# nicolasavru/objective-slam

Hardware: AMD Instinct MI355X
Metric: scene_ppf_votes_per_sec (higher is better)
Workload: dtype f32; 1 GPU; 5k-point model vs 100k-point scene (BASELINE.json metric config), one resident model table, Model::ppf_lookup per step; model_points=5000, scene_points=100000, ref_point_df=8, ref_points_per_gpu=12500, vote_mode=exact, parallelism=scene-ref-shard x1, exchange=single GPU

## Files before the change

include/oslam.h:

```cpp
#ifndef OSLAM_H
#define OSLAM_H

#include <stddef.h>
#include <stdint.h>

#ifdef __cplusplus
extern "C" {
#endif

#define OSLAM_OK 0
#define OSLAM_E_INVALID 1
#define OSLAM_E_DEVICE 2
#define OSLAM_E_NOMEM 3
#define OSLAM_E_NO_VOTES 4
#define OSLAM_E_LIMIT 5
#define OSLAM_E_PEER 6

#define OSLAM_VOTE_EXACT 0
#define OSLAM_VOTE_FAST 1

typedef struct oslam_params {
    unsigned ref_point_df;
    float vote_count_threshold;
    int cpu_clustering;
    int use_l1_norm;
    int use_averaged_clusters;
    int dev;
    int vote_mode;
    int shard_rank;
    int shard_world;
    unsigned max_cells;
    unsigned pose_gpu_min;
    int no_bucket_spread;
    unsigned scratch_gib;
    int pose_two_sorts;
    int vote_order;
    int reserved[1];
} oslam_params;

typedef struct oslam_stats {
    uint64_t num_scene_ppfs;
    uint64_t num_hits;
    uint64_t num_votes;
    uint64_t num_unique_votes;
    uint64_t num_model_keys;
    uint64_t num_top;
    uint32_t max_count;
    uint32_t num_emitted;
    float ms_vote;
    float ms_total;
    uint32_t vote_launches;
    float ms_vote_kernel;
    float ms_key_kernel;
    uint32_t wide_workgroups;
    uint64_t num_pairs_probed;
    uint64_t scratch_bytes;
    uint64_t num_entries_streamed;
    uint64_t num_items;
} oslam_stats;

typedef struct oslam_cell {
    uint64_t code;
    uint32_t count;
    uint32_t pad;
} oslam_cell;

typedef struct oslam_model oslam_model;
typedef struct oslam_scene oslam_scene;

int oslam_params_default(oslam_params *p);

int oslam_d_dist_from_cloud(const float *xyz, size_t n, size_t stride_bytes, float tau_d,
                            float *d_dist_out);

int oslam_model_create(const float *xyz, const float *nrm, size_t n, size_t stride_bytes,
                       float d_dist, const oslam_params *params, oslam_model **out);
void oslam_model_destroy(oslam_model *m);

int oslam_model_save(const oslam_model *m, const char *path);
int oslam_model_load(const char *path, const oslam_params *params, oslam_model **out);
int oslam_model_info(const oslam_model *m, size_t *n_points, float *d_dist, uint64_t *table_bytes);

int oslam_model_set_point_weights(oslam_model *m, const float *weights, size_t n);

int oslam_scene_create(const float *xyz, const float *nrm, size_t n, size_t stride_bytes,
                       float d_dist, unsigned ref_point_downsample_factor,
                       const oslam_params *params, oslam_scene **out);
void oslam_scene_destroy(oslam_scene *s);

int oslam_align(oslam_model *m, oslam_scene *s, float T_rowmajor[16], oslam_stats *stats);

int oslam_align_prepare(oslam_model *m, oslam_scene *s);

typedef struct oslam_db oslam_db;
int oslam_db_create(oslam_model *const *models, size_t n, oslam_db **out);
void oslam_db_destroy(oslam_db *db);
void oslam_db_destroy_with_models(oslam_db *db);
int oslam_db_align(oslam_db *db, oslam_scene *s, float *T_out, oslam_stats *stats);
int oslam_db_size(const oslam_db *db, size_t *n_models, size_t *n_groups);

int oslam_ppf_registration(const float *const *scene_xyz, const float *const *scene_nrm,
                           const size_t *scene_n, size_t n_scenes, const float *const *model_xyz,
                           const float *const *model_nrm, const size_t *model_n, size_t n_models,
                           size_t stride_bytes, const float *model_d_dists,
                           unsigned ref_point_downsample_factor, float vote_count_threshold,
                           int cpu_clustering, int use_l1_norm, int use_averaged_clusters, int devUse,
                           const float *model_weights, float *T_out);

int oslam_ht_dist(const float A[16], const float B[16], float out[2]);

int oslam_voxel_grid(const float *xyz, const float *nrm, size_t n, size_t stride_bytes, float leaf,
                     int dev, float *xyz_out, float *nrm_out, size_t cap, size_t *n_out);

typedef struct oslam_camera {
    float fx, fy, cx, cy;
    float depth_scale;
    float z_min, z_max;
    float max_jump;
} oslam_camera;
int oslam_depth_to_cloud(const void *depth, int depth_is_u16, int width, int height, const oslam_camera *cam,
// ... 563 lines not shown
int oslam_world_bricks(oslam_world *w, int32_t *keys_out, size_t cap, size_t *n_out);
int oslam_scene_from_world(oslam_world *w, oslam_volume *vol, const oslam_world_surface_params *sp, float leaf, float d_dist,
                           unsigned ref_point_downsample_factor, const oslam_params *params, oslam_scene **out,
                           size_t *n_points_out);

typedef struct oslam_world_mesh_result {
    uint32_t vertices;
    uint32_t triangles;
    uint32_t cubes;
    uint32_t bricks;
    uint32_t window_bricks;
    uint32_t launches;
    int32_t anchor[3];
    float ms_total;
} oslam_world_mesh_result;

int oslam_world_mesh(oslam_world *w, oslam_volume *vol, const oslam_world_surface_params *sp, float *xyz_out, float *nrm_out,
                     int32_t *key_out, size_t v_cap, uint32_t *tri_out, size_t t_cap, size_t *nv_out, size_t *nt_out,
                     oslam_world_mesh_result *res);

#define OSLAM_NORMALS_SWEEPS 4
typedef struct oslam_normals_params {
    float radius;
    unsigned min_neighbours;
    float viewpoint[3];
    int orient;
    float line_ratio;
    int reserved[4];
} oslam_normals_params;

typedef struct oslam_normals_result {
    uint32_t n_valid;
    uint32_t n_cells;
    float edge;
    uint32_t launches;
    float ms_total;
    float ms_grid, ms_kernel;
} oslam_normals_result;

int oslam_normals_params_default(oslam_normals_params *p);
int oslam_cloud_normals(const float *xyz, size_t n, size_t stride_bytes, const oslam_normals_params *np, int dev,
                        float *nrm_out, float *curvature_out, uint8_t *valid_out, oslam_normals_result *res);
int oslam_cloud_normal_moments(const float *xyz, size_t n, size_t stride_bytes, const oslam_normals_params *np, int dev,
                               int64_t *moments_out);
int oslam_mesh_normals(const float *xyz, size_t nv, size_t stride_bytes, const uint32_t *tri, size_t nt, float *nrm_out,
                       uint8_t *valid_out);
int oslam_ply_read_mesh(const char *path, float **xyz_out, float **nrm_out, uint32_t **tri_out, size_t *nv_out,
                        size_t *nt_out);

typedef struct oslam_colour_params {
    unsigned max_weight;
    float band;
    int reserved[6];
} oslam_colour_params;

int oslam_view_set_colour(oslam_view *v, const uint8_t *rgb, size_t row_stride_bytes, const uint8_t *valid);
int oslam_view_colour(oslam_view *v, uint32_t *rgba_out);
int oslam_view_has_colour(const oslam_view *v);
int oslam_colour_params_default(oslam_colour_params *p);
int oslam_volume_colour_enable(oslam_volume *vol, const oslam_colour_params *cp);
int oslam_volume_colour_words(oslam_volume *vol, uint32_t *words_out);
int oslam_volume_set_colour_words(oslam_volume *vol, const uint32_t *words);
int oslam_volume_integrate_colour(oslam_volume *vol, const oslam_view *v, const oslam_view *c, const float T_vol_cam[16],
                                  oslam_integrate_result *res, uint32_t *coloured_out);
int oslam_volume_colours(oslam_volume *vol, const float *xyz, size_t n, size_t stride_bytes, uint8_t *rgb_out,
                         uint8_t *valid_out, size_t *n_valid_out);
int oslam_volume_paint_view(oslam_volume *vol, const float T_vol_cam[16], oslam_view *v, uint32_t *painted_out);
int oslam_ply_write_colour(const char *path, const float *xyz, const float *nrm, const uint8_t *rgb, size_t n, int binary);
int oslam_ply_write_mesh_colour(const char *path, const float *xyz, const float *nrm, const uint8_t *rgb, size_t nv,
                                const uint32_t *tri, size_t nt, int binary);
int oslam_world_colours(oslam_world *w, oslam_volume *vol, const oslam_world_surface_params *sp, const float *xyz, size_t n,
                        size_t stride_bytes, uint8_t *rgb_out, uint8_t *valid_out, size_t *n_valid_out);

int oslam_scene_keys(oslam_scene *s, size_t ref_index, uint32_t *keys_out);
int oslam_model_keys(oslam_model *m, size_t ref_index, uint32_t *keys_out);
int oslam_model_bucket(oslam_model *m, uint32_t key, uint32_t *pairs_out, size_t cap,
                       size_t *count_out);
int oslam_model_bucket_words(oslam_model *m, uint32_t key, int slice, uint32_t *words_out, size_t cap,
                             size_t *count_out);
int oslam_model_key_numbers(oslam_model *m, uint32_t *keys_out, uint32_t *numbers_out, uint64_t *weights_out, size_t cap,
                            size_t *n_out);
int oslam_vote_ref_order(const uint32_t *keep, size_t n, uint32_t *order_out);
int oslam_vote_accumulator(oslam_model *m, oslam_scene *s, size_t ref_index, uint32_t *acc_out);
int oslam_vote_hits(oslam_model *m, oslam_scene *s, size_t ref_index, uint32_t *numbers_out, uint32_t *theta_out,
                    uint32_t *idx_out, size_t cap, size_t *n_out, uint32_t *keep_out);
int oslam_last_cells(oslam_model *m, oslam_cell *cells_out, float *poses_out, size_t cap,
                     size_t *n_out);

int oslam_set_stream(void *hip_stream);
int oslam_release_scratch(int dev);
const char *oslam_last_error(void);
int oslam_set_host_threads(int n);
int oslam_selftest_math(size_t n, uint64_t seed, uint64_t *mismatches);

#ifdef __cplusplus
}
#endif
#endif
```

objective-slam_amd/csrc/oslam_host.c:

```c
#include <pthread.h>
#include <stdio.h>

#include "oslam_internal.h"

static __thread char g_err[512];
static __thread void *g_stream;

const char *oslam_last_error(void) { return g_err; }

int oslam_set_stream(void *hip_stream)
{
    g_stream = hip_stream;
    return OSLAM_OK;
}

void *oslam_stream(void) { return g_stream; }

int oslam_fail(int code, const char *what)
{
    if (what != g_err) snprintf(g_err, sizeof g_err, "%s", what);
    return code;
}

int oslam_fail_call(const char *call, int err, const char *file, int line)
{
    snprintf(g_err, sizeof g_err, "%s: %s (%s:%d)", call, hipGetErrorString((hipError_t)err), file, line);
    return OSLAM_E_DEVICE;
}

int oslam_params_default(oslam_params *p)
{
    if (!p) return fail(OSLAM_E_INVALID, "params is NULL");
    memset(p, 0, sizeof *p);
    p->ref_point_df = 1;
    p->vote_count_threshold = 0.4f;
    p->cpu_clustering = 0;
    p->use_l1_norm = 0;
    p->use_averaged_clusters = 0;
    p->dev = 0;
    p->vote_mode = OSLAM_VOTE_EXACT;
    p->shard_rank = 0;
    p->shard_world = 1;
    p->max_cells = 1u << 22;
    p->pose_gpu_min = 0;
    p->no_bucket_spread = 0;
    p->scratch_gib = 0;
    p->vote_order = 0;
    return OSLAM_OK;
}

int oslam_d_dist_from_cloud(const float *xyz, size_t n, size_t stride_bytes, float tau_d,
                            float *d_dist_out)
{
    float lo[3], hi[3], ext;
    size_t i;
    int a;
    if (!xyz || !d_dist_out || n == 0 || stride_bytes < 12) return fail(OSLAM_E_INVALID, "bad cloud");
    for (a = 0; a < 3; a++) lo[a] = hi[a] = xyz[a];
    for (i = 1; i < n; i++) {
        const float *p = (const float *)((const char *)xyz + i * stride_bytes);
        for (a = 0; a < 3; a++) {
            if (p[a] < lo[a]) lo[a] = p[a];
            if (p[a] > hi[a]) hi[a] = p[a];
        }
    }
    ext = hi[0] - lo[0];
    if (hi[1] - lo[1] > ext) ext = hi[1] - lo[1];
    if (hi[2] - lo[2] > ext) ext = hi[2] - lo[2];
    *d_dist_out = tau_d * ext;
    return OSLAM_OK;
}

int oslam_pick_device(int dev_req, int *dev_out)
{
    int n = 0;
    hipError_t e = hipGetDeviceCount(&n);
    if (e != hipSuccess || n <= 0) return fail(OSLAM_E_DEVICE, "no HIP device available (the PPF path has no CPU fallback)");
    if (dev_req < 0) dev_req = 0;
    *dev_out = dev_req < n - 1 ? dev_req : n - 1;
    e = hipSetDevice(*dev_out);
    if (e != hipSuccess) return fail(OSLAM_E_DEVICE, hipGetErrorString(e));
    return OSLAM_OK;
}

#define DEVCACHE_SLOTS 64
#define DEVCACHE_MAX_BLOCK ((size_t)1 << 30)
typedef struct {
    void *p;
    size_t bytes;
    int dev, used;
} devblock;
static devblock g_devcache[DEVCACHE_SLOTS];
static pthread_mutex_t g_devcache_mu = PTHREAD_MUTEX_INITIALIZER;

int oslam_dev_alloc(void **out, size_t bytes)
{
    int dev = 0, i, best = -1, spare = -1;
    hipError_t e;
    size_t want;
    *out = NULL;
    if (bytes == 0) bytes = 16;
    if (hipGetDevice(&dev) != hipSuccess) return (int)hipErrorInvalidDevice;
    pthread_mutex_lock(&g_devcache_mu);
    for (i = 0; i < DEVCACHE_SLOTS; i++) {
        devblock *b = &g_devcache[i];
        if (!b->p) { if (spare < 0) spare = i; continue; }
        if (b->used || b->dev != dev || b->bytes < bytes || b->bytes > 2 * bytes + 65536) continue;
        if (best < 0 || b->bytes < g_devcache[best].bytes) best = i;
    }
    if (best >= 0) {
        g_devcache[best].used = 1;
        *out = g_devcache[best].p;
        pthread_mutex_unlock(&g_devcache_mu);
        return 0;
    }
    want = bytes <= DEVCACHE_MAX_BLOCK ? bytes + bytes / 8 + 256 : bytes;
    e = hipMalloc(out, want);
    if (e != hipSuccess) {
        (void)hipGetLastError();
        for (i = 0; i < DEVCACHE_SLOTS; i++)
            if (g_devcache[i].p && !g_devcache[i].used && g_devcache[i].dev == dev) {
                (void)hipFree(g_devcache[i].p);
                memset(&g_devcache[i], 0, sizeof g_devcache[i]);
                if (spare < 0) spare = i;
            }
        want = bytes;
        e = hipMalloc(out, want);
    }
    if (e == hipSuccess && spare >= 0 && want <= DEVCACHE_MAX_BLOCK) {
        g_devcache[spare].p = *out;
// ... 35 lines not shown
```

objective-slam_amd/csrc/oslam_internal.h:

```cpp
#ifndef OSLAM_INTERNAL_H
#define OSLAM_INTERNAL_H

#include <hip/hip_runtime_api.h>
#include <limits.h>
#include <stddef.h>
#include <stdint.h>
#include <stdlib.h>
#include <string.h>
#include <time.h>

#include "oslam.h"
#include "oslam_kernels.h"
#include "oslam_rigid.h"

typedef struct cloud_buf {
    int n;
    float *h_xyz, *h_nrm;
    float *d_soa;
    oslamk_cloud k;
} cloud_buf;

struct oslam_model {
    int dev;
    cloud_buf c;
    float d_dist, inv_d_dist;
    oslam_params params;
    oslamk_table table;
    oslamk_entries ent;
    uint32_t n_entries;
    uint64_t num_model_keys;
    float *weights;
    oslamk_counters *d_counters;
    oslamk_cell *d_out;
    uint32_t out_cap;
    oslam_cell *h_out;
    size_t n_local;
    uint32_t local_max;
    oslamk_cell *d_union;
    size_t union_cap;
    float *d_Tm16, *d_weights;
    oslam_cell *last_cells;
    float *last_poses;
    size_t n_last;
    int last_on_device;
    oslamk_cell *d_pose_cells;
    float *d_pose_T;
    size_t pose_cap;
    oslamk_slot *h_slots;
    int shared_union;
    int unusable;
    double cm[3];
    float inst_c[3], inst_extent;
    double bound_r;
    int bound_set;
};

struct oslam_scene {
    int dev;
    cloud_buf c;
    float d_dist;
    unsigned df;
    int rank, world;
    int n_ref;
    uint32_t *h_ref_idx, *d_ref_idx;
    float *d_tsg;
    float *d_Ts16;
    uint32_t *d_block;
    oslamk_order order;
    struct oslam_scene_grid *grids;
};

struct oslam_view {
    int dev;
    oslamk_view k;
    float *d_z;
    float max_jump;
    float *d_maps;
    uint32_t *d_colour;
};

struct oslam_volume {
    int dev;
    oslamk_volume k;
    oslam_volume_params p;
    int off[3];
    uint32_t *spare;
    oslamk_colour colour;
    uint32_t *colour_spare;
};

struct oslam_pyramid {
    int dev;
    unsigned n_levels;
    oslam_view *level[3];
};

struct oslam_render {
    int dev;
    oslam_view *view;
    size_t n_hyp;
    int32_t *d_labels;
    float *d_tol;
};

typedef struct db_group {
    int n;
    size_t *members;
    uint32_t *ukeys, *reach, *kmap, *uids;
} db_group;

struct oslam_db {
    int dev;
    size_t n;
// ... 166 lines not shown
```

objective-slam_amd/csrc/oslam_kernels.h:

```cpp
#ifndef OSLAM_KERNELS_H
#define OSLAM_KERNELS_H

#include <stddef.h>
#include <stdint.h>

#ifdef __cplusplus
extern "C" {
#endif

#define OSLAMK_SLICE 2046
#define OSLAMK_ROWS 1024
#define OSLAMK_NBIN 32

typedef struct oslamk_slot {
    uint32_t key;
    uint32_t start;
    uint32_t len;
    uint32_t cur;
} oslamk_slot;

typedef struct oslamk_uv {
    float uy, uz;
} oslamk_uv;

typedef struct oslamk_entries {
    uint32_t *e4;
    oslamk_uv *uv;
    uint16_t *mi;
    uint32_t *pw;
    oslamk_uv *puv;
    uint16_t *pdir;
    uint32_t n_real;
} oslamk_entries;
#define OSLAMK_PSEG 4096
#ifndef OSLAMK_PDIR_SHIFT
#define OSLAMK_PDIR_SHIFT 0
#endif
#define OSLAMK_PDIR_CELLS_RAW(m) ((m) <= 1u ? 1u : 1u << (31 - __builtin_clz((m) - 1u)))
#define OSLAMK_PDIR_CELLS(n) (OSLAMK_PDIR_CELLS_RAW((n) << OSLAMK_PDIR_SHIFT) > 4096u ? 4096u : OSLAMK_PDIR_CELLS_RAW((n) << OSLAMK_PDIR_SHIFT))

typedef struct oslamk_cloud {
    const float *px, *py, *pz, *nx, *ny, *nz;
    int n;
} oslamk_cloud;

typedef struct oslamk_order {
    const float *sx, *sy, *sz;
    const uint32_t *perm;
    const float *box;
} oslamk_order;
#define OSLAMK_ORDER_GROUP 64

typedef struct oslamk_uinfo {
    uint32_t start;
    uint32_t len;
} oslamk_uinfo;

typedef struct oslamk_table {
    oslamk_slot *slots;
    uint32_t cap;
    uint32_t shift;
    int n_slices;
    uint32_t *ukeys;
    uint32_t ucap;
    uint32_t ushift;
    uint32_t *reach;
    uint32_t reach_words;
    uint32_t *kmap;
    uint32_t kmap_bins;
    uint32_t *uids;
    uint32_t n_ids, id_bits, uinfo_stride;
    oslamk_uinfo *uinfo;
} oslamk_table;
#define OSLAMK_UWEIGHTS(t) ((unsigned long long *)((t).uids + (t).ucap))
#define OSLAMK_KMAP_NONE 0xffffffffu
#define OSLAMK_KMAP_MAX_BINS 2048

#define OSLAMK_REACH_BINS 16384

typedef struct oslamk_counters {
    unsigned long long hits;
    unsigned long long votes;
    unsigned long long nonzero_cells;
    uint32_t gmax;
    uint32_t out_count;
    uint32_t redo_count;
    uint32_t redo_total;
    unsigned long long entries;
    unsigned long long items;
    unsigned long long prof[4];
    uint32_t list_overflow;
    uint32_t pad_;
} oslamk_counters;

typedef struct oslamk_cell {
    unsigned long long code;
    uint32_t count;
    uint32_t pad;
} oslamk_cell;

int oslamk_row_keys(oslamk_cloud c, int ref, float d_dist, float inv_d_dist, uint32_t *keys_out,
                    void *stream);

int oslamk_model_count(oslamk_cloud c, float d_dist, float inv_d_dist, oslamk_table t,
                       uint32_t *n_unique, uint32_t *overflow, void *stream);
int oslamk_table_scan(oslamk_table t, uint32_t *total_out, void *stream);
int oslamk_union_build(oslamk_table t, uint32_t *n_keys, uint32_t *overflow, void *stream);
int oslamk_reach_build(oslamk_table t, float d_dist, void *stream);
int oslamk_union_weights(oslamk_table t, unsigned long long *weights, void *stream);
int oslamk_kmap_build(oslamk_table t, float d_dist, void *stream);
int oslamk_model_fill(oslamk_cloud c, float d_dist, float inv_d_dist, oslamk_table t,
                      const float *tmg, oslamk_entries ent, void *stream);

int oslamk_bucket_spread(oslamk_table t, oslamk_entries ent, void *stream);
int oslamk_bucket_psort(oslamk_table t, oslamk_entries ent, void *stream);

typedef struct oslamk_pay {
    uint32_t theta_t22;
    uint32_t idx;
} oslamk_pay;

typedef struct oslamk_run {
    uint32_t slot_r;
    uint32_t first;
} oslamk_run;
#define OSLAMK_RUN_SHIFT 26

typedef struct oslamk_vote_args {
    oslamk_cloud scene;
    const uint32_t *ref_idx;
    const float *tsg;
    int n_ref;
    float d_dist, inv_d_dist;
    oslamk_table table;
    oslamk_entries ent;
    float thresh;
    uint32_t fixed_gmax;
    oslamk_counters *counters;
    oslamk_cell *out;
    uint32_t out_cap;
    uint32_t *acc_dump;
    int dump_ref;
    int first_ref;
    int n_launch;
    int mode;
    uint32_t *keep_count;
    const uint32_t *hit_off;
    uint32_t *hit_key;
    oslamk_pay *hit_pay;
    oslamk_pay *hit_sorted;
    oslamk_run *runs;
    uint32_t *hit_count;
    uint32_t *run_count;
    uint32_t *redo;
    const uint32_t *ref_order;
    oslamk_order order;
} oslamk_vote_args;

int oslamk_uinfo_build(oslamk_table t, void *stream);

int oslamk_scene_count(const oslamk_vote_args *a, void *stream);
int oslamk_scene_hits(const oslamk_vote_args *a, void *stream);
int oslamk_sort_hits(const oslamk_vote_args *a, void *stream);
int oslamk_vote(const oslamk_vote_args *a, void *stream);
int oslamk_vote_wide(const oslamk_vote_args *a, void *stream);
int oslamk_vote_group(const oslamk_vote_args *d_all, const oslamk_vote_args *h_all, int nm, void *stream);

int oslamk_voxel_grid(oslamk_cloud c, float leaf, float *out6, uint32_t *n_out, void *stream);

int oslamk_depth_to_cloud(const void *d_img, int is_u16, int w, int h, float fx, float fy, float cx, float cy,
                          float scale, float z_min, float z_max, float max_jump, float *d_out6, uint32_t *n_out,
                          void *stream);

int oslam_dev_alloc(void **p, size_t bytes);
void oslam_dev_free(void *p);
void oslam_dev_cache_release(int dev);

int oslamk_aos6_to_soa(const float *d_in6, size_t n, float *d_soa, void *stream);

int oslamk_cluster_scores(int n, const int *cell, const uint32_t *shash, const uint32_t *sidx,
                          const float *sq, const float *st, const float *sw, float d_dist, int use_l1,
                          float *score, int whole_host, const unsigned long long *whole_dev, uint32_t *table, void *stream);
size_t oslamk_cluster_table_words(int n);

#define OSLAMK_MAX_INSTANCES 64
typedef struct oslamk_inst_args {
    uint32_t max_instances;
    float ratio, sep2, cos_thr;
    int32_t rot_on;
    float c[3];
} oslamk_inst_args;
typedef struct oslamk_inst_out {
    uint32_t n;
    uint32_t idx[OSLAMK_MAX_INSTANCES];
    float score[OSLAMK_MAX_INSTANCES];
    float T[OSLAMK_MAX_INSTANCES][16];
} oslamk_inst_out;

// ... 361 lines not shown
```

objective-slam_amd/csrc/oslam_kernels.hip:

```cpp
#include <hip/hip_runtime.h>

#include "oslam_kernels.h"
#include "ppf_core.h"

#include "oslam_vote_body.inc"

__device__ __forceinline__ uint32_t slot_of(uint32_t key, uint32_t shift)
{
    return (key * 2654435761u) >> shift;
}

__device__ __forceinline__ uint32_t cloud_pair_key(const oslamk_cloud &c, int i, float prx,
                                                   float pry, float prz, float nrx, float nry,
                                                   float nrz, float nrn, float d_dist,
                                                   float inv_d_dist, float *pix, float *piy,
                                                   float *piz)
{
    float px = c.px[i], py = c.py[i], pz = c.pz[i];
    float nx = c.nx[i], ny = c.ny[i], nz = c.nz[i];
    *pix = px;
    *piy = py;
    *piz = pz;
    return pc_pair_key(prx, pry, prz, nrx, nry, nrz, nrn, px, py, pz, nx, ny, nz,
                       pc_norm3(nx, ny, nz), d_dist, inv_d_dist);
// ... 246 lines not shown
                key[i] = ((unsigned long long)spread_key(w) << 32) | i;
            } else {
                key[i] = ~0ull;
            }
        }
        __syncthreads();
        for (uint32_t k = 2; k <= P; k <<= 1) {
            for (uint32_t j = k >> 1; j > 0; j >>= 1) {
                for (uint32_t x = tid; x < P / 2; x += SPREAD_THREADS) {
                    const uint32_t lo = ((x & ~(j - 1)) << 1) | (x & (j - 1)), hi = lo | j;
                    const unsigned long long a = key[lo], b = key[hi];
                    const bool up = (lo & k) == 0;
                    if ((a > b) == up) { key[lo] = b; key[hi] = a; }
                }
                __syncthreads();
            }
        }
        const uint32_t n_full = n >> 8, n_last = n & 255u;
        for (uint32_t p = tid; p < n; p += SPREAD_THREADS) {
            const uint32_t c = p >> 8, q = p & 255u, h = (q >> 2) & 31u;
            const uint32_t nc = c < n_full ? 256u : n_last;
            uint32_t rank = 8u * h * n_full + spread_rank_in_chunk(4u * h, n_last);
            rank += 8u * (c < n_full ? c : n_full);
            rank += spread_rank_in_chunk(q, nc) - spread_rank_in_chunk(4u * h, nc);
            const uint32_t src = (uint32_t)key[rank];
            ent.e4[base + p] = s_e4[src];
            if (ent.uv) ent.uv[base + p] = s_uv[src];
            ent.mi[base + p] = s_mi[src];
        }
        __syncthreads();
    }
}

__global__ __launch_bounds__(SPREAD_THREADS) void k_bucket_psort(oslamk_table t, oslamk_entries ent)
{
    __shared__ unsigned long long key[OSLAMK_PSEG];
    __shared__ uint32_t s_e4[OSLAMK_PSEG];
    __shared__ oslamk_uv s_uv[OSLAMK_PSEG];
    const oslamk_slot sl = t.slots[blockIdx.x];
    if (sl.key == 0 || sl.len == 0) return;
    const int tid = threadIdx.x;
    for (uint32_t seg = 0; seg < sl.len; seg += OSLAMK_PSEG) {
        const uint32_t n = sl.len - seg < OSLAMK_PSEG ? sl.len - seg : OSLAMK_PSEG;
        const size_t base = (size_t)sl.start + seg;
        uint32_t P = 2;
        while (P < n) P <<= 1;
        for (uint32_t i = tid; i < P; i += SPREAD_THREADS) {
            if (i < n) {
                const uint32_t w = ent.e4[base + i];
                s_e4[i] = w;
                s_uv[i] = ent.uv[base + i];
                key[i] = ((unsigned long long)(w * 30u) << 32) | i;
            } else {
                key[i] = ~0ull;
            }
        }
        __syncthreads();
        for (uint32_t k = 2; k <= P; k <<= 1) {
            for (uint32_t j = k >> 1; j > 0; j >>= 1) {
                for (uint32_t x = tid; x < P / 2; x += SPREAD_THREADS) {
                    const uint32_t lo = ((x & ~(j - 1)) << 1) | (x & (j - 1)), hi = lo | j;
                    const unsigned long long a = key[lo], b = key[hi];
                    const bool up = (lo & k) == 0;
                    if ((a > b) == up) { key[lo] = b; key[hi] = a; }
                }
                __syncthreads();
            }
        }
        for (uint32_t i = tid; i < n; i += SPREAD_THREADS) {
            const uint32_t src = (uint32_t)key[i];
            ent.pw[base + i] = s_e4[src];
            ent.puv[base + i] = s_uv[src];
        }
        const uint32_t K = OSLAMK_PDIR_CELLS(n);
        for (uint32_t k = tid; k <= K; k += SPREAD_THREADS) {
            uint32_t lo = 0, hi = n;
            while (lo < hi) {
                const uint32_t mid = (lo + hi) >> 1;
                const uint32_t cell = (uint32_t)(((key[mid] >> 32) * (unsigned long long)K) >> 32);
                if (cell < k) lo = mid + 1; else hi = mid;
            }
            ent.pdir[(base << OSLAMK_PDIR_SHIFT) + k] = (uint16_t)lo;
        }
        __syncthreads();
    }
}

#define KEY_TILE 4096
#define COUNT_REFS 8
#define HIT_TILE 1024

__device__ const uint32_t d_acos_lut[2 * PC_ACOS_CELLS] = {PC_ACOS_LUT_FLAT};

__device__ __forceinline__ int pair_dist_bin_quick(float dx, float dy, float dz, float d_dist, float inv_d_dist)
{
    const float d2 = dx * dx + dy * dy + dz * dz;
    const float q = __builtin_amdgcn_sqrtf(d2) * inv_d_dist;
    const float kf = __builtin_floorf(q);
    const float fr = q - kf, tol = q * 1e-6f;
    int k = (int)kf;
    if (!(d2 > 1e-30f && q < 1048576.0f && fr > tol && 1.0f - fr > tol)) k = pc_pair_dist_bin(dx, dy, dz, d_dist, inv_d_dist);
    return k;
}

__device__ __forceinline__ bool bin_in_reach(const uint32_t *reach, uint32_t reach_words, int k)
{
    if ((uint32_t)k >= OSLAMK_REACH_BINS) return true;
    const uint32_t w = (uint32_t)k >> 5;
    return w < reach_words && ((reach[w] >> ((uint32_t)k & 31u)) & 1u);
}

struct KeyRefs {
    uint32_t rr[COUNT_REFS];
    float prx[COUNT_REFS], pry[COUNT_REFS], prz[COUNT_REFS];
};
__device__ __forceinline__ void key_refs_load(KeyRefs &r, const oslamk_vote_args &a, int g0)
{
#pragma unroll
    for (int g = 0; g < COUNT_REFS; g++) {
        const bool v = g0 + g < a.n_launch;
        r.rr[g] = v ? a.ref_idx[a.first_ref + g0 + g] : 0xffffffffu;
        r.prx[g] = v ? a.scene.px[r.rr[g]] : 0.0f;
        r.pry[g] = v ? a.scene.py[r.rr[g]] : 0.0f;
        r.prz[g] = v ? a.scene.pz[r.rr[g]] : 0.0f;
    }
}
__device__ __forceinline__ void reach_fill(uint32_t *s_reach, const uint32_t *reach, uint32_t reach_words)
{
    for (uint32_t w = threadIdx.x; w < reach_words; w += 256) s_reach[w] = reach[w];
}
__device__ __forceinline__ bool pair_keep(const KeyRefs &r, int g, bool valid, int i, bool in, float x, float y, float z,
                                          const oslamk_vote_args &a, const uint32_t *s_reach, uint32_t reach_words)
{
    const int k = pair_dist_bin_quick(x - r.prx[g], y - r.pry[g], z - r.prz[g], a.d_dist, a.inv_d_dist);
    return in && (uint32_t)i != r.rr[g] && valid && bin_in_reach(s_reach, reach_words, k);
}

__device__ __forceinline__ bool range_in_reach(const uint32_t *reach, uint32_t reach_words, int kmin, int kmax)
{
    if (kmax >= OSLAMK_REACH_BINS) return true;
    const uint32_t w0 = (uint32_t)kmin >> 5, w1 = (uint32_t)kmax >> 5;
    for (uint32_t w = w0; w <= w1 && w < reach_words; w++) {
        uint32_t m = reach[w];
        if (w == w0) m &= 0xffffffffu << ((uint32_t)kmin & 31u);
        if (w == w1) m &= 0xffffffffu >> (31u - ((uint32_t)kmax & 31u));
        if (m) return true;
    }
    return false;
}
__device__ __forceinline__ bool group_keep(const oslamk_vote_args &a, int g, int grp, const uint32_t *s_reach, uint32_t reach_words)
{
    if (g >= a.n_launch || grp * OSLAMK_ORDER_GROUP >= a.scene.n) return false;
#ifdef KEY_DIAG_KEEP_ALL
    return true;
#endif
    const uint32_t rr = a.ref_idx[a.first_ref + g];
    int kmin, kmax;
    if (!pc_box_bin_range(a.order.box + 6 * (size_t)grp, a.scene.px[rr], a.scene.py[rr], a.scene.pz[rr], a.inv_d_dist, &kmin, &kmax))
        return true;
    return range_in_reach(s_reach, reach_words, kmin, kmax);
}

__global__ __launch_bounds__(256) void k_scene_count(oslamk_vote_args a)
{
    __shared__ uint32_t s_cnt[COUNT_REFS];
    __shared__ uint32_t s_reach[OSLAMK_REACH_BINS / 32];
// ... 325 lines not shown
        for (int k = 0; k < 4; k++) {
            if ((uint32_t)k >= G) continue;
            float v = votes;
            if (whole) {
                float s = lane_sum[k];
                for (int o = WAVE / 2; o > 0; o >>= 1) s += __shfl_xor(s, o, WAVE);
                v = 1 + s;
            }
            if (lane == 0) score[orig[k]] = v;
        }
        g0 += G;
    }
}

__global__ void k_selftest(const float *x, const float *y, const float *x2, size_t n, float *out_acos,
                           float *out_atan2, uint32_t *out_quant, uint32_t *out_bin)
{
    __shared__ uint32_t s_tbl[32];
    if (threadIdx.x < 32) s_tbl[threadIdx.x] = k_alpha_thr[threadIdx.x];
    __syncthreads();
    size_t i = (size_t)blockIdx.x * blockDim.x + threadIdx.x;
    if (i >= n) return;
    out_acos[i] = pm_acosf(x[i]);
    out_atan2[i] = pm_atan2f(y[i], x2[i]);
    out_quant[i] = pc_quant_bits(pm_fabsf(y[i]) * 7.0f, 0.0371f + pm_fabsf(x[i]) * 0.01f,
                                 1.0f / (0.0371f + pm_fabsf(x[i]) * 0.01f));
    out_bin[i] = pc_alpha_bin_table(y[i], x2[i], x[i], y[i] - x2[i], s_tbl);
}

extern "C" {

int oslamk_row_keys(oslamk_cloud c, int ref, float d_dist, float inv_d_dist, uint32_t *keys_out,
                    void *stream)
{
    hipLaunchKernelGGL(k_row_keys, dim3((c.n + 255) / 256), dim3(256), 0, (hipStream_t)stream, c, ref,
                       d_dist, inv_d_dist, keys_out);
    return (int)hipGetLastError();
}

int oslamk_model_count(oslamk_cloud c, float d_dist, float inv_d_dist, oslamk_table t,
                       uint32_t *n_unique, uint32_t *overflow, void *stream)
{
    hipLaunchKernelGGL(k_model_count, dim3((c.n + 255) / 256, c.n), dim3(256), 0, (hipStream_t)stream,
                       c, d_dist, inv_d_dist, t, n_unique, overflow);
    return (int)hipGetLastError();
}

int oslamk_table_scan(oslamk_table t, uint32_t *total_out, void *stream)
{
    hipLaunchKernelGGL(k_table_scan, dim3(1), dim3(1024), 0, (hipStream_t)stream, t, total_out);
    return (int)hipGetLastError();
}

int oslamk_union_build(oslamk_table t, uint32_t *n_keys, uint32_t *overflow, void *stream)
{
    size_t total = (size_t)t.n_slices * t.cap;
    hipLaunchKernelGGL(k_union_build, dim3((unsigned)((total + 255) / 256)), dim3(256), 0,
                       (hipStream_t)stream, t, n_keys, overflow);
    return (int)hipGetLastError();
}

int oslamk_model_fill(oslamk_cloud c, float d_dist, float inv_d_dist, oslamk_table t,
                      const float *tmg, oslamk_entries ent, void *stream)
{
    hipLaunchKernelGGL(k_model_fill, dim3((c.n + 255) / 256, c.n), dim3(256), 0, (hipStream_t)stream,
                       c, d_dist, inv_d_dist, t, tmg, ent);
    return (int)hipGetLastError();
}

int oslamk_bucket_spread(oslamk_table t, oslamk_entries ent, void *stream)
{
    const size_t total = (size_t)t.n_slices * t.cap;
    hipLaunchKernelGGL(k_bucket_spread, dim3((unsigned)total), dim3(SPREAD_THREADS), 0, (hipStream_t)stream, t, ent);
    return (int)hipGetLastError();
}

int oslamk_bucket_psort(oslamk_table t, oslamk_entries ent, void *stream)
{
    const size_t total = (size_t)t.n_slices * t.cap;
    hipLaunchKernelGGL(k_bucket_psort, dim3((unsigned)total), dim3(SPREAD_THREADS), 0, (hipStream_t)stream, t, ent);
    return (int)hipGetLastError();
}

int oslamk_reach_build(oslamk_table t, float d_dist, void *stream)
{
    hipLaunchKernelGGL(k_reach_build, dim3(OSLAMK_REACH_BINS), dim3(256), 0, (hipStream_t)stream, t, d_dist);
    return (int)hipGetLastError();
}

int oslamk_union_weights(oslamk_table t, unsigned long long *weights, void *stream)
{
    const size_t total = (size_t)t.n_slices * t.cap;
    hipLaunchKernelGGL(k_union_weights, dim3((unsigned)((total + 255) / 256)), dim3(256), 0, (hipStream_t)stream, t, weights);
    return (int)hipGetLastError();
}

int oslamk_kmap_build(oslamk_table t, float d_dist, void *stream)
{
    if (t.kmap_bins == 0) return 0;
    hipLaunchKernelGGL(k_kmap_build, dim3(t.kmap_bins), dim3(256), 0, (hipStream_t)stream, t, d_dist);
    return (int)hipGetLastError();
}

int oslamk_uinfo_build(oslamk_table t, void *stream)
{
    const size_t total = (size_t)t.n_slices * t.cap;
    hipLaunchKernelGGL(k_uinfo_build, dim3((unsigned)((total + 255) / 256)), dim3(256), 0, (hipStream_t)stream, t);
    return (int)hipGetLastError();
}

int oslamk_scene_count(const oslamk_vote_args *a, void *stream)
{
    if (a->n_launch <= 0) return 0;
    dim3 grid((unsigned)((a->n_launch + COUNT_REFS - 1) / COUNT_REFS), (unsigned)((a->scene.n + KEY_TILE - 1) / KEY_TILE));
    hipLaunchKernelGGL(k_scene_count, grid, dim3(256), 0, (hipStream_t)stream, *a);
    return (int)hipGetLastError();
}

int oslamk_scene_hits(const oslamk_vote_args *a, void *stream)
{
    if (a->n_launch <= 0) return 0;
    dim3 grid((unsigned)((a->n_launch + COUNT_REFS - 1) / COUNT_REFS), (unsigned)((a->scene.n + HIT_TILE - 1) / HIT_TILE));
    hipLaunchKernelGGL(k_scene_hits, grid, dim3(256), 0, (hipStream_t)stream, *a);
    return (int)hipGetLastError();
}


int oslamk_vote(const oslamk_vote_args *a, void *stream)
{
    if (a->n_launch <= 0) return 0;
    dim3 grid((unsigned)(((size_t)a->n_launch + 7) / 8 * 8 * a->table.n_slices));
    hipLaunchKernelGGL((a->mode == 0 ? k_vote<0> : k_vote<1>), grid, dim3(VOTE_THREADS), 0, (hipStream_t)stream, *a);
    return oslamk_vote_wide(a, stream);
}

int oslamk_vote_group(const oslamk_vote_args *d_all, const oslamk_vote_args *h_all, int nm, void *stream)
{
    if (nm <= 0 || h_all[0].n_launch <= 0) return 0;
    int max_slices = 1;
    for (int j = 0; j < nm; j++) {
        if (h_all[j].n_launch != h_all[0].n_launch || h_all[j].mode != h_all[0].mode) return (int)hipErrorInvalidValue;
        if (h_all[j].table.n_slices > max_slices) max_slices = h_all[j].table.n_slices;
    }
    const size_t wgs = ((size_t)h_all[0].n_launch + 7) / 8 * 8 * (size_t)max_slices;
    if (wgs * (size_t)nm > 0x7fffffffu) return (int)hipErrorInvalidValue;
    hipLaunchKernelGGL((h_all[0].mode == 0 ? k_vote_group<0> : k_vote_group<1>), dim3((unsigned)(wgs * (size_t)nm)),
                       dim3(VOTE_THREADS), 0, (hipStream_t)stream, d_all, (uint32_t)wgs);
    return (int)hipGetLastError();
}

size_t oslamk_cluster_table_words(int n)
{
    uint32_t cap = 64;
    while (cap < 2u * (uint32_t)(n > 0 ? n : 1)) cap <<= 1;
    return 3u * (size_t)cap;
}

int oslamk_cluster_scores(int n, const int *cell, const uint32_t *shash, const uint32_t *sidx,
                          const float *sq, const float *st, const float *sw, float d_dist, int use_l1,
                          float *score, int whole_host, const unsigned long long *whole_dev, uint32_t *table, void *stream)
{
    if (n <= 0) return 0;
    const size_t words = oslamk_cluster_table_words(n);
    const uint32_t mask = (uint32_t)(words / 3u) - 1u;
    hipError_t e = hipMemsetAsync(table, 0, sizeof(uint32_t) * words, (hipStream_t)stream);
    if (e != hipSuccess) return (int)e;
// ... 34 lines not shown
```

objective-slam_amd/csrc/oslam_model.c:

```c
#include <stdio.h>

#include "oslam_internal.h"
#include "oslam_pose.h"
#include "ppf_core.h"

void oslam_model_destroy(oslam_model *m)
{
    if (!m) return;
    (void)hipSetDevice(m->dev);
    oslam_cloud_free(&m->c);
    if (m->table.slots) (void)hipFree(m->table.slots);
    if (m->ent.e4) (void)hipFree(m->ent.e4);
    if (m->ent.uv) (void)hipFree(m->ent.uv);
    if (m->ent.pw) (void)hipFree(m->ent.pw);
    if (m->ent.puv) (void)hipFree(m->ent.puv);
    if (m->ent.pdir) (void)hipFree(m->ent.pdir);
    if (m->ent.mi) (void)hipFree(m->ent.mi);
    if (m->table.ukeys && !m->shared_union) (void)hipFree(m->table.ukeys);
    if (m->table.reach && !m->shared_union) (void)hipFree(m->table.reach);
    if (m->table.kmap && !m->shared_union) (void)hipFree(m->table.kmap);
    if (m->table.uids && !m->shared_union) (void)hipFree(m->table.uids);
    if (m->d_counters) (void)hipFree(m->d_counters);
    if (m->d_out) (void)hipFree(m->d_out);
    if (m->d_union) (void)hipFree(m->d_union);
    if (m->table.uinfo) (void)hipFree(m->table.uinfo);
    if (m->d_Tm16) (void)hipFree(m->d_Tm16);
    if (m->d_weights) (void)hipFree(m->d_weights);
    if (m->d_pose_cells) (void)hipFree(m->d_pose_cells);
    if (m->d_pose_T) (void)hipFree(m->d_pose_T);
    free(m->h_out);
    free(m->weights);
    free(m->last_cells);
    free(m->last_poses);
    free(m->h_slots);
    free(m);
}

typedef struct key_rank {
    uint64_t weight;
    uint32_t key, slot;
} key_rank;

static void rank_pass(const key_rank *src, key_rank *dst, size_t n, int by_weight, unsigned shift, uint32_t *count)
{
    size_t i;
    uint32_t run = 0, d;
    memset(count, 0, sizeof(uint32_t) * 65536);
    for (i = 0; i < n; i++) {
        d = by_weight ? 0xffffu - (uint32_t)((src[i].weight >> shift) & 0xffffu) : (src[i].key >> shift) & 0xffffu;
        count[d]++;
    }
    for (d = 0; d < 65536; d++) {
        const uint32_t c = count[d];
        count[d] = run;
        run += c;
    }
    for (i = 0; i < n; i++) {
        d = by_weight ? 0xffffu - (uint32_t)((src[i].weight >> shift) & 0xffffu) : (src[i].key >> shift) & 0xffffu;
        dst[count[d]++] = src[i];
    }
}

static key_rank *rank_keys(key_rank *r, key_rank *tmp, size_t n, uint32_t *count)
{
    uint64_t top = 0;
    unsigned shift;
    size_t i;
    key_rank *t;
    for (i = 0; i < n; i++) if (r[i].weight > top) top = r[i].weight;
    for (shift = 0; shift < 32; shift += 16) {
        rank_pass(r, tmp, n, 0, shift, count);
        t = r; r = tmp; tmp = t;
    }
    for (shift = 0; shift < 64 && (top >> shift); shift += 16) {
        rank_pass(r, tmp, n, 1, shift, count);
        t = r; r = tmp; tmp = t;
    }
    return r;
}

int oslam_build_kmap(oslamk_table *t, float d_dist, const oslamk_table *parts, int n_parts, int vote_order)
{
    int rc = OSLAM_OK, j;
    uint32_t h_reach[OSLAMK_REACH_BINS / 32], w, top = 0, n_ids = 0, slot;
    uint32_t *h_keys = NULL, *h_ids = NULL, *count = NULL;
    uint64_t *h_w = NULL;
    key_rank *r = NULL, *r2 = NULL, *res;
    const size_t ucap = t->ucap;
    const int ranked = vote_order == 0 || vote_order == 2;
    t->kmap = NULL;
    t->kmap_bins = 0;
    t->reach_words = 0;
    t->uids = NULL;
    t->n_ids = t->id_bits = t->uinfo_stride = 0;
    HIPCHK(hipMalloc((void **)&t->uids, (sizeof(uint32_t) + sizeof(uint64_t)) * ucap));
    HIPCHK(hipMemsetAsync(t->uids, 0, (sizeof(uint32_t) + sizeof(uint64_t)) * ucap, (hipStream_t)oslam_stream()));
    for (j = 0; j < n_parts; j++) {
        oslamk_table p = parts[j];
        p.ukeys = t->ukeys;
// ... 18 lines not shown
        for (slot = 0; slot < ucap; slot++)
            if (h_keys[slot] != 0u) {
                r[i].weight = h_w[slot];
                r[i].key = h_keys[slot];
                r[i].slot = slot;
                i++;
            }
        res = rank_keys(r, r2, n_ids, count);
        for (i = 0; i < n_ids; i++) h_ids[res[i].slot] = (uint32_t)i;
    } else {
        uint32_t next = 0;
        for (slot = 0; slot < ucap; slot++)
            if (h_keys[slot] != 0u) h_ids[slot] = next++;
    }
    HIPCHK(hipMemcpy(t->uids, h_ids, sizeof(uint32_t) * ucap, hipMemcpyHostToDevice));
    t->n_ids = n_ids;
    t->id_bits = 1;
    while (t->id_bits < 32u && ((uint64_t)1 << t->id_bits) < (uint64_t)n_ids) t->id_bits++;
    t->uinfo_stride = (n_ids + 63u) & ~63u;
    if (t->uinfo_stride == 0) t->uinfo_stride = 64;
    HIPCHK(hipMemcpy(h_reach, t->reach, sizeof h_reach, hipMemcpyDeviceToHost));
    for (w = 0; w < OSLAMK_REACH_BINS / 32; w++)
        if (h_reach[w]) {
            t->reach_words = w + 1;
            top = 32u * w + (32u - (uint32_t)__builtin_clz(h_reach[w]));
        }
    t->kmap_bins = top < OSLAMK_KMAP_MAX_BINS ? top : OSLAMK_KMAP_MAX_BINS;
    if (t->kmap_bins) {
        HIPCHK(hipMalloc((void **)&t->kmap, sizeof(uint32_t) * (size_t)t->kmap_bins * PC_ANGLE_COMBOS));
        KCHK(oslamk_kmap_build(*t, d_dist, oslam_stream()));
    }
done:
    free(h_keys);
    free(h_ids);
    free(h_w);
    free(count);
    free(r);
    free(r2);
    return rc;
}

int oslam_build_union(oslam_model *m, uint32_t distinct, uint32_t *d_n_keys, uint32_t *d_overflow)
{
    int rc = OSLAM_OK;
    uint32_t lg = 16;
    while ((1u << lg) < 4u * distinct && lg < OSLAMK_RUN_SHIFT) lg++;
    if ((1u << lg) < 2u * distinct) return fail(OSLAM_E_LIMIT, "more distinct pair keys than the union table can index");
    if (m->table.ukeys && !m->shared_union) (void)hipFree(m->table.ukeys);
    if (m->table.reach && !m->shared_union) (void)hipFree(m->table.reach);
    if (m->table.kmap && !m->shared_union) (void)hipFree(m->table.kmap);
    if (m->table.uids && !m->shared_union) (void)hipFree(m->table.uids);
    m->table.ukeys = NULL;
    m->table.reach = NULL;
    m->table.kmap = NULL;
    m->table.uids = NULL;
    m->shared_union = 0;
    m->table.ucap = 1u << lg;
    m->table.ushift = 32 - lg;
    HIPCHK(hipMalloc((void **)&m->table.ukeys, sizeof(uint32_t) * (size_t)m->table.ucap));
    HIPCHK(hipMemsetAsync(m->table.ukeys, 0, sizeof(uint32_t) * (size_t)m->table.ucap, (hipStream_t)oslam_stream()));
    HIPCHK(hipMemsetAsync(d_overflow, 0, sizeof(uint32_t), (hipStream_t)oslam_stream()));
    HIPCHK(hipMemsetAsync(d_n_keys, 0, sizeof(uint32_t), (hipStream_t)oslam_stream()));
    KCHK(oslamk_union_build(m->table, d_n_keys, d_overflow, oslam_stream()));
    HIPCHK(hipMalloc((void **)&m->table.reach, sizeof(uint32_t) * (OSLAMK_REACH_BINS / 32)));
    HIPCHK(hipMemsetAsync(m->table.reach, 0, sizeof(uint32_t) * (OSLAMK_REACH_BINS / 32), (hipStream_t)oslam_stream()));
    KCHK(oslamk_reach_build(m->table, m->d_dist, oslam_stream()));
    rc = oslam_build_kmap(&m->table, m->d_dist, &m->table, 1, m->params.vote_order);
done:
    return rc;
}

int oslam_build_uinfo(oslam_model *m)
{
    int rc = OSLAM_OK;
    const size_t bytes = sizeof(oslamk_uinfo) * (size_t)m->table.n_slices * (size_t)m->table.uinfo_stride;
    if (m->table.uinfo) { (void)hipFree(m->table.uinfo); m->table.uinfo = NULL; }
    HIPCHK(hipMalloc((void **)&m->table.uinfo, bytes));
    HIPCHK(hipMemsetAsync(m->table.uinfo, 0, bytes, (hipStream_t)oslam_stream()));
    KCHK(oslamk_uinfo_build(m->table, oslam_stream()));
done:
    return rc;
}

int oslam_model_create(const float *xyz, const float *nrm, size_t n, size_t stride_bytes,
                       float d_dist, const oslam_params *params, oslam_model **out)
{
    int rc = OSLAM_OK;
    oslam_model *m = NULL;
    uint32_t *d_small = NULL;
    uint32_t h_small[64 + 3];
    float *h_tmg = NULL, *d_tmg = NULL;
    int n_slices, s;
    uint32_t cap;
    size_t n_pairs;

    if (!out) return fail(OSLAM_E_INVALID, "out is NULL");
    *out = NULL;
    if (!xyz || !nrm || stride_bytes < 12 || !(d_dist > 0.0f)) return fail(OSLAM_E_INVALID, "bad model arguments");
    if (n < 2) return fail(OSLAM_E_INVALID, "model needs at least 2 points");
    if (n > 46340) return fail(OSLAM_E_LIMIT, "model larger than 46340 points (32-bit pair index, kernel.cu:433)");
    m = (oslam_model *)calloc(1, sizeof *m);
    if (!m) return fail(OSLAM_E_NOMEM, "host allocation failed");
    if (params) m->params = *params; else oslam_params_default(&m->params);
    if (m->params.max_cells == 0) m->params.max_cells = 1u << 22;
    rc = oslam_pick_device(m->params.dev, &m->dev);
    if (rc != OSLAM_OK) goto done;
    rc = oslam_cloud_make(&m->c, xyz, nrm, stride_bytes, NULL, n);
    if (rc != OSLAM_OK) goto done;
    oslam_cloud_shape(m->c.h_xyz, n, m->cm, m->inst_c, &m->inst_extent);
    m->d_dist = d_dist;
    m->inv_d_dist = 1.0f / d_dist;
    m->weights = (float *)malloc(sizeof(float) * n);
    if (!m->weights) { rc = fail(OSLAM_E_NOMEM, "host allocation failed"); goto done; }
    for (s = 0; s < (int)n; s++) m->weights[s] = 1.0f;

    n_slices = (int)((n + OSLAMK_SLICE - 1) / OSLAMK_SLICE);
    if (n_slices > 64) { rc = fail(OSLAM_E_LIMIT, "too many model slices"); goto done; }
    HIPCHK(hipMalloc((void **)&d_small, sizeof(uint32_t) * (64 + 3)));

    for (cap = 1u << 16;; cap <<= 1) {
        int grow = 0;
        uint32_t lg = 0;
        while ((1u << lg) < cap) lg++;
        if (m->table.slots) { (void)hipFree(m->table.slots); m->table.slots = NULL; }
        HIPCHK(hipMalloc((void **)&m->table.slots, sizeof(oslamk_slot) * (size_t)cap * n_slices));
        HIPCHK(hipMemsetAsync(m->table.slots, 0, sizeof(oslamk_slot) * (size_t)cap * n_slices, (hipStream_t)oslam_stream()));
        HIPCHK(hipMemsetAsync(d_small, 0, sizeof(uint32_t) * (64 + 3), (hipStream_t)oslam_stream()));
        m->table.cap = cap;
        m->table.shift = 32 - lg;
        m->table.n_slices = n_slices;
        KCHK(oslamk_model_count(m->c.k, m->d_dist, m->inv_d_dist, m->table, d_small, d_small + 64, oslam_stream()));
        HIPCHK(hipStreamSynchronize((hipStream_t)oslam_stream()));
        HIPCHK(hipMemcpy(h_small, d_small, sizeof h_small, hipMemcpyDeviceToHost));
        if (h_small[64]) grow = 1;
        for (s = 0; s < n_slices; s++) if (h_small[s] > cap / 2) grow = 1;
        if (!grow) break;
        if (cap >= (1u << 26)) { rc = fail(OSLAM_E_LIMIT, "model hash table would exceed 2^26 slots per slice"); goto done; }
    }
    KCHK(oslamk_table_scan(m->table, d_small + 65, oslam_stream()));
    {
        uint32_t sum = 0;
        for (s = 0; s < n_slices; s++) sum += h_small[s];
        rc = oslam_build_union(m, sum, d_small + 66, d_small + 64);
        if (rc != OSLAM_OK) goto done;
    }
    HIPCHK(hipStreamSynchronize((hipStream_t)oslam_stream()));
    HIPCHK(hipMemcpy(h_small, d_small, sizeof h_small, hipMemcpyDeviceToHost));
    if (h_small[64]) { rc = fail(OSLAM_E_LIMIT, "union key table overflow"); goto done; }
    m->n_entries = h_small[65];
    m->ent.n_real = m->n_entries;
    m->num_model_keys = (uint64_t)h_small[66] + 1;
    n_pairs = m->n_entries ? m->n_entries : 1;

    h_tmg = (float *)malloc(sizeof(float) * 8 * n);
    if (!h_tmg) { rc = fail(OSLAM_E_NOMEM, "host allocation failed"); goto done; }
    oslam_T_g_rows(m->c.h_xyz, m->c.h_nrm, NULL, n, h_tmg);
    HIPCHK(hipMalloc((void **)&d_tmg, sizeof(float) * 8 * n));
    HIPCHK(hipMemcpy(d_tmg, h_tmg, sizeof(float) * 8 * n, hipMemcpyHostToDevice));
    HIPCHK(hipMalloc((void **)&m->ent.e4, sizeof(uint32_t) * (n_pairs + 256)));
    HIPCHK(hipMalloc((void **)&m->ent.mi, sizeof(uint16_t) * n_pairs));
    if (m->params.vote_mode != OSLAM_VOTE_FAST)
        HIPCHK(hipMalloc((void **)&m->ent.uv, sizeof(oslamk_uv) * n_pairs));
    HIPCHK(hipMemsetD32Async((hipDeviceptr_t)m->ent.e4, (int)PC_ROW_SINK, n_pairs + 256, (hipStream_t)oslam_stream()));
    KCHK(oslamk_model_fill(m->c.k, m->d_dist, m->inv_d_dist, m->table, d_tmg, m->ent, oslam_stream()));
    if (!m->params.no_bucket_spread) KCHK(oslamk_bucket_spread(m->table, m->ent, oslam_stream()));
    if (m->ent.uv) {
        HIPCHK(hipMalloc((void **)&m->ent.pw, sizeof(uint32_t) * n_pairs));
        HIPCHK(hipMalloc((void **)&m->ent.puv, sizeof(oslamk_uv) * n_pairs));
        HIPCHK(hipMalloc((void **)&m->ent.pdir, sizeof(uint16_t) * ((n_pairs + 256) << OSLAMK_PDIR_SHIFT)));
        KCHK(oslamk_bucket_psort(m->table, m->ent, oslam_stream()));
        HIPCHK(hipStreamSynchronize((hipStream_t)oslam_stream()));
        (void)hipFree(m->ent.uv);
        m->ent.uv = NULL;
    }
    rc = oslam_build_uinfo(m);
    if (rc != OSLAM_OK) goto done;
    HIPCHK(hipStreamSynchronize((hipStream_t)oslam_stream()));

    m->out_cap = m->params.max_cells;
    HIPCHK(hipMalloc((void **)&m->d_counters, sizeof(oslamk_counters)));
    HIPCHK(hipMalloc((void **)&m->d_out, sizeof(oslamk_cell) * (size_t)m->out_cap));
    m->h_out = (oslam_cell *)malloc(sizeof(oslam_cell) * (size_t)m->out_cap);
    if (!m->h_out) { rc = fail(OSLAM_E_NOMEM, "host allocation failed"); goto done; }
done:
    free(h_tmg);
    if (d_tmg) (void)hipFree(d_tmg);
    if (d_small) (void)hipFree(d_small);
    if (rc != OSLAM_OK) { oslam_model_destroy(m); return rc; }
    *out = m;
    return OSLAM_OK;
}

#define OSLAM_DB_MAGIC 0x4c444d4f534c4f00ull
#define OSLAM_DB_VERSION 7u
typedef struct db_header {
    uint64_t magic;
    uint32_t version, vote_mode;
    uint32_t n_points, n_slices, cap, shift, ucap, ushift, n_entries, has_uv;
    uint64_t num_model_keys;
    float d_dist, inv_d_dist;
    uint64_t checksum;
} db_header;

static uint64_t fnv64(uint64_t h, const void *p, size_t n)
{
    const unsigned char *b = (const unsigned char *)p;
    size_t i;
    for (i = 0; i < n; i++) { h ^= b[i]; h *= 0x100000001b3ull; }
    return h;
}

static int db_write_dev(FILE *f, const void *dev, size_t bytes, uint64_t *sum)
{
    int rc = OSLAM_OK;
    const size_t chunk = (size_t)64 << 20;
    char *h = (char *)malloc(bytes < chunk ? (bytes ? bytes : 1) : chunk);
    size_t off;
    if (!h) return fail(OSLAM_E_NOMEM, "host allocation failed");
    for (off = 0; off < bytes; off += chunk) {
        const size_t n = bytes - off < chunk ? bytes - off : chunk;
        HIPCHK(hipMemcpy(h, (const char *)dev + off, n, hipMemcpyDeviceToHost));
        *sum = fnv64(*sum, h, n);
        if (fwrite(h, 1, n, f) != n) { rc = fail(OSLAM_E_INVALID, "short write"); goto done; }
    }
done:
    free(h);
    return rc;
}

static int db_read_dev(FILE *f, void *dev, size_t bytes, uint64_t *sum)
{
    int rc = OSLAM_OK;
    const size_t chunk = (size_t)64 << 20;
    char *h = (char *)malloc(bytes < chunk ? (bytes ? bytes : 1) : chunk);
    size_t off;
    if (!h) return fail(OSLAM_E_NOMEM, "host allocation failed");
    for (off = 0; off < bytes; off += chunk) {
        const size_t n = bytes - off < chunk ? bytes - off : chunk;
        if (fread(h, 1, n, f) != n) { rc = fail(OSLAM_E_INVALID, "model file is truncated"); goto done; }
        *sum = fnv64(*sum, h, n);
        HIPCHK(hipMemcpy((char *)dev + off, h, n, hipMemcpyHostToDevice));
    }
done:
    free(h);
    return rc;
}

static uint32_t log2_exact(uint32_t v)
{
    uint32_t lg = 0;
    while ((1u << lg) < v) lg++;
    return lg;
}
// ... 72 lines not shown
        hd.ucap > (1u << OSLAMK_RUN_SHIFT) || hd.shift != 32u - log2_exact(hd.cap) || hd.ushift != 32u - log2_exact(hd.ucap) ||
        !(hd.d_dist > 0.0f) || hd.inv_d_dist != 1.0f / hd.d_dist || hd.has_uv > 1u ||
        hd.vote_mode > (uint32_t)OSLAM_VOTE_FAST || (hd.vote_mode != (uint32_t)OSLAM_VOTE_FAST && !hd.has_uv) ||
        (uint64_t)hd.n_entries > (uint64_t)n * (n - 1) + 3ull * (uint64_t)hd.cap * hd.n_slices ||
        hd.num_model_keys > (uint64_t)hd.ucap + 1) {
        rc = fail(OSLAM_E_INVALID, "model file header is inconsistent");
        goto done;
    }
    hz = hd;
    hz.checksum = 0;
    sum = fnv64(sum, &hz, sizeof hz);
    m = (oslam_model *)calloc(1, sizeof *m);
    if (!m) { rc = fail(OSLAM_E_NOMEM, "host allocation failed"); goto done; }
    if (params) m->params = *params; else oslam_params_default(&m->params);
    if (m->params.max_cells == 0) m->params.max_cells = 1u << 22;
    if (params && (uint32_t)params->vote_mode != hd.vote_mode && !(hd.has_uv && params->vote_mode == OSLAM_VOTE_FAST)) {
        rc = fail(OSLAM_E_INVALID, "model file was built in fast vote mode: it has no exact entries");
        goto done;
    }
    if (!params) m->params.vote_mode = (int)hd.vote_mode;
    rc = oslam_pick_device(m->params.dev, &m->dev);
    if (rc != OSLAM_OK) goto done;
    xyz = (float *)malloc(12 * n);
    nrm = (float *)malloc(12 * n);
    m->weights = (float *)malloc(4 * n);
    n_slots = (size_t)hd.cap * hd.n_slices;
    h_slots = (oslamk_slot *)malloc(sizeof(oslamk_slot) * n_slots);
    if (!xyz || !nrm || !m->weights || !h_slots) { rc = fail(OSLAM_E_NOMEM, "host allocation failed"); goto done; }
    if (fread(xyz, 12, n, f) != n || fread(nrm, 12, n, f) != n || fread(m->weights, 4, n, f) != n ||
        fread(h_slots, sizeof(oslamk_slot), n_slots, f) != n_slots) {
        rc = fail(OSLAM_E_INVALID, "model file is truncated");
        goto done;
    }
    sum = fnv64(sum, xyz, 12 * n);
    sum = fnv64(sum, nrm, 12 * n);
    sum = fnv64(sum, m->weights, 4 * n);
    sum = fnv64(sum, h_slots, sizeof(oslamk_slot) * n_slots);
    {
        uint64_t run = 0;
        for (i = 0; i < n_slots; i++) {
            if (h_slots[i].start != run || run + h_slots[i].len > hd.n_entries) {
                rc = fail(OSLAM_E_INVALID, "model file: a bucket lies outside the entry arrays or out of order");
                goto done;
            }
            run += ((uint64_t)h_slots[i].len + 3u) & ~(uint64_t)3u;
        }
    }
    rc = oslam_cloud_make(&m->c, xyz, nrm, 12, NULL, n);
    if (rc != OSLAM_OK) goto done;
    oslam_cloud_shape(m->c.h_xyz, n, m->cm, m->inst_c, &m->inst_extent);
    m->d_dist = hd.d_dist;
    m->inv_d_dist = hd.inv_d_dist;
    m->table.cap = hd.cap;
    m->table.shift = hd.shift;
    m->table.n_slices = (int)hd.n_slices;
    m->table.ucap = hd.ucap;
    m->table.ushift = hd.ushift;
    m->n_entries = hd.n_entries;
    m->ent.n_real = hd.n_entries;
    m->num_model_keys = hd.num_model_keys;
    n_pairs = hd.n_entries ? hd.n_entries : 1;
    HIPCHK(hipMalloc((void **)&m->table.slots, sizeof(oslamk_slot) * n_slots));
    HIPCHK(hipMalloc((void **)&m->table.ukeys, sizeof(uint32_t) * (size_t)hd.ucap));
    HIPCHK(hipMalloc((void **)&m->table.reach, sizeof(uint32_t) * (OSLAMK_REACH_BINS / 32)));
    HIPCHK(hipMalloc((void **)&m->ent.e4, sizeof(uint32_t) * (n_pairs + 256)));
    HIPCHK(hipMalloc((void **)&m->ent.mi, sizeof(uint16_t) * n_pairs));
    if (hd.has_uv) {
        HIPCHK(hipMalloc((void **)&m->ent.pw, sizeof(uint32_t) * n_pairs));
        HIPCHK(hipMalloc((void **)&m->ent.puv, sizeof(oslamk_uv) * n_pairs));
        HIPCHK(hipMalloc((void **)&m->ent.pdir, sizeof(uint16_t) * ((n_pairs + 256) << OSLAMK_PDIR_SHIFT)));
    }
    HIPCHK(hipMemcpy(m->table.slots, h_slots, sizeof(oslamk_slot) * n_slots, hipMemcpyHostToDevice));
    HIPCHK(hipMemsetD32Async((hipDeviceptr_t)m->ent.e4, (int)PC_ROW_SINK, n_pairs + 256, (hipStream_t)oslam_stream()));
    HIPCHK(hipStreamSynchronize((hipStream_t)oslam_stream()));
    rc = db_read_dev(f, m->table.ukeys, sizeof(uint32_t) * (size_t)hd.ucap, &sum);
    if (rc == OSLAM_OK) rc = db_read_dev(f, m->table.reach, sizeof(uint32_t) * (OSLAMK_REACH_BINS / 32), &sum);
    if (rc == OSLAM_OK) rc = db_read_dev(f, m->ent.e4, sizeof(uint32_t) * (size_t)hd.n_entries, &sum);
    if (rc == OSLAM_OK) rc = db_read_dev(f, m->ent.mi, sizeof(uint16_t) * (size_t)hd.n_entries, &sum);
    if (rc == OSLAM_OK && hd.has_uv) rc = db_read_dev(f, m->ent.pw, sizeof(uint32_t) * (size_t)hd.n_entries, &sum);
    if (rc == OSLAM_OK && hd.has_uv) rc = db_read_dev(f, m->ent.puv, sizeof(oslamk_uv) * (size_t)hd.n_entries, &sum);
    if (rc == OSLAM_OK && hd.has_uv) rc = db_read_dev(f, m->ent.pdir, sizeof(uint16_t) * ((size_t)hd.n_entries << OSLAMK_PDIR_SHIFT), &sum);
    if (rc != OSLAM_OK) goto done;
    if (sum != hd.checksum) { rc = fail(OSLAM_E_INVALID, "model file checksum mismatch"); goto done; }
    m->h_slots = h_slots;
    h_slots = NULL;
    rc = oslam_build_kmap(&m->table, m->d_dist, &m->table, 1, m->params.vote_order);
    if (rc != OSLAM_OK) goto done;
    rc = oslam_build_uinfo(m);
    if (rc != OSLAM_OK) goto done;
    HIPCHK(hipStreamSynchronize((hipStream_t)oslam_stream()));
    m->out_cap = m->params.max_cells;
    HIPCHK(hipMalloc((void **)&m->d_counters, sizeof(oslamk_counters)));
    HIPCHK(hipMalloc((void **)&m->d_out, sizeof(oslamk_cell) * (size_t)m->out_cap));
    m->h_out = (oslam_cell *)malloc(sizeof(oslam_cell) * (size_t)m->out_cap);
    if (!m->h_out) { rc = fail(OSLAM_E_NOMEM, "host allocation failed"); goto done; }
done:
    if (f) fclose(f);
    free(xyz);
    free(nrm);
    free(h_slots);
    if (rc != OSLAM_OK) { oslam_model_destroy(m); return rc; }
    *out = m;
    return OSLAM_OK;
}

int oslam_model_info(const oslam_model *m, size_t *n_points, float *d_dist, uint64_t *table_bytes)
{
    if (!m) return fail(OSLAM_E_INVALID, "NULL handle");
    if (n_points) *n_points = (size_t)m->c.n;
    if (d_dist) *d_dist = m->d_dist;
    if (table_bytes)
        *table_bytes = sizeof(oslamk_slot) * (uint64_t)m->table.cap * (uint64_t)m->table.n_slices +
                       sizeof(uint32_t) * (uint64_t)m->table.ucap + sizeof(uint32_t) * (OSLAMK_REACH_BINS / 32) +
                       sizeof(oslamk_uinfo) * (uint64_t)m->table.uinfo_stride * (uint64_t)m->table.n_slices +
                       (uint64_t)m->n_entries * (4 + 2 + (m->ent.pw ? 12 + (2 << OSLAMK_PDIR_SHIFT) : 0)) + 24ull * (uint64_t)m->c.n;
    return OSLAM_OK;
}

int oslam_model_set_point_weights(oslam_model *m, const float *weights, size_t n)
{
    if (!m || !weights || n != (size_t)m->c.n) return fail(OSLAM_E_INVALID, "bad weights");
    memcpy(m->weights, weights, sizeof(float) * n);
    if (m->d_weights) {
        if (hipSetDevice(m->dev) != hipSuccess ||
            hipMemcpy(m->d_weights, m->weights, sizeof(float) * n, hipMemcpyHostToDevice) != hipSuccess)
            return fail(OSLAM_E_DEVICE, "cannot update the weights on the device");
    }
    return OSLAM_OK;
}
```

objective-slam_amd/csrc/oslam_taps.c:

```c

#include "oslam_internal.h"
#include "oslam_pose.h"
#include "ppf_core.h"

static int cloud_row_keys(cloud_buf *c, size_t ref, float d_dist, uint32_t *keys_out)
{
    int rc = OSLAM_OK;
    uint32_t *d = NULL;
    if (!keys_out || ref >= (size_t)c->n) return fail(OSLAM_E_INVALID, "bad reference index");
    HIPCHK(hipMalloc((void **)&d, sizeof(uint32_t) * c->n));
    KCHK(oslamk_row_keys(c->k, (int)ref, d_dist, 1.0f / d_dist, d, oslam_stream()));
    HIPCHK(hipStreamSynchronize((hipStream_t)oslam_stream()));
    HIPCHK(hipMemcpy(keys_out, d, sizeof(uint32_t) * c->n, hipMemcpyDeviceToHost));
done:
    if (d) (void)hipFree(d);
    return rc;
}

int oslam_scene_keys(oslam_scene *s, size_t ref_index, uint32_t *keys_out)
{
    if (!s) return fail(OSLAM_E_INVALID, "NULL handle");
    if (!(s->d_dist > 0.0f)) return fail(OSLAM_E_INVALID, "this scene was made for models of any d_dist (d_dist 0): it has no keys of its own");
    if (hipSetDevice(s->dev) != hipSuccess) return fail(OSLAM_E_DEVICE, "hipSetDevice failed");
    return cloud_row_keys(&s->c, ref_index, s->d_dist, keys_out);
// ... 112 lines not shown
    h_w = (uint64_t *)malloc(sizeof(uint64_t) * ucap);
    rows = (key_row *)malloc(sizeof *rows * ucap);
    if (!h_keys || !h_ids || !h_w || !rows) { rc = fail(OSLAM_E_NOMEM, "host allocation failed"); goto done; }
    HIPCHK(hipMemcpy(h_keys, m->table.ukeys, sizeof(uint32_t) * ucap, hipMemcpyDeviceToHost));
    HIPCHK(hipMemcpy(h_ids, m->table.uids, sizeof(uint32_t) * ucap, hipMemcpyDeviceToHost));
    HIPCHK(hipMemcpy(h_w, OSLAMK_UWEIGHTS(m->table), sizeof(uint64_t) * ucap, hipMemcpyDeviceToHost));
    for (slot = 0; slot < ucap; slot++)
        if (h_keys[slot] != 0u) {
            rows[n].key = h_keys[slot];
            rows[n].number = h_ids[slot];
            rows[n].weight = h_w[slot];
            n++;
        }
    qsort(rows, n, sizeof *rows, key_row_order);
    for (i = 0; i < n && i < cap; i++) {
        if (keys_out) keys_out[i] = rows[i].key;
        if (numbers_out) numbers_out[i] = rows[i].number;
        if (weights_out) weights_out[i] = rows[i].weight;
    }
    *n_out = n;
done:
    free(h_keys);
    free(h_ids);
    free(h_w);
    free(rows);
    return rc;
}

int oslam_vote_ref_order(const uint32_t *keep, size_t n, uint32_t *order_out)
{
    if ((!keep || !order_out) && n) return fail(OSLAM_E_INVALID, "NULL argument");
    oslam_ref_order(keep, n, order_out);
    return OSLAM_OK;
}

static int tap_one_ref(oslam_model *m, oslam_scene *s, size_t ref_index, uint32_t *acc_out, uint32_t *numbers_out,
                       uint32_t *theta_out, uint32_t *idx_out, size_t cap, size_t *n_out, uint32_t *keep_out)
{
    int rc = OSLAM_OK;
    uint32_t *d_dump = NULL, *d_ref = NULL, *h_dump = NULL;
    float *d_tsg = NULL;
    float rows[8];
    uint32_t ref = (uint32_t)ref_index;
    oslamk_counters cnt;
    scratch_pool *pool = NULL;
    size_t cells;
    rc = oslam_check_pair(m, s);
    if (rc != OSLAM_OK) return rc;
    if (ref_index >= (size_t)s->c.n) return fail(OSLAM_E_INVALID, "bad reference index");
    cells = (size_t)m->table.n_slices * OSLAMK_SLICE * OSLAMK_NBIN;
    oslam_T_g_rows(s->c.h_xyz, s->c.h_nrm, &ref, 1, rows);
    rc = oslam_pool_enter(m->dev, &pool);
    if (rc != OSLAM_OK) return rc;
    HIPCHK(hipMalloc((void **)&d_dump, sizeof(uint32_t) * cells));
    HIPCHK(hipMalloc((void **)&d_ref, sizeof(uint32_t)));
    HIPCHK(hipMalloc((void **)&d_tsg, sizeof rows));
    HIPCHK(hipMemcpy(d_ref, &ref, sizeof ref, hipMemcpyHostToDevice));
    HIPCHK(hipMemcpy(d_tsg, rows, sizeof rows, hipMemcpyHostToDevice));
    rc = oslam_run_votes_group(pool, &m, 1, s, d_ref, d_tsg, 1, 0xffffffffu, d_dump, &cnt, NULL);
    if (rc != OSLAM_OK) goto done;
    if (n_out) {
        rc = oslam_pool_read_hits(pool, numbers_out, theta_out, idx_out, cap, n_out, keep_out);
        if (rc != OSLAM_OK) goto done;
    }
    if (acc_out) {
        h_dump = (uint32_t *)malloc(sizeof(uint32_t) * cells);
        if (!h_dump) { rc = fail(OSLAM_E_NOMEM, "host allocation failed"); goto done; }
        HIPCHK(hipMemcpy(h_dump, d_dump, sizeof(uint32_t) * cells, hipMemcpyDeviceToHost));
        memcpy(acc_out, h_dump, sizeof(uint32_t) * OSLAMK_NBIN * (size_t)m->c.n);
    }
done:
    oslam_pool_unlock(pool);
    free(h_dump);
    if (d_dump) (void)hipFree(d_dump);
    if (d_ref) (void)hipFree(d_ref);
    if (d_tsg) (void)hipFree(d_tsg);
    return rc;
}

int oslam_vote_accumulator(oslam_model *m, oslam_scene *s, size_t ref_index, uint32_t *acc_out)
{
    if (!acc_out) return fail(OSLAM_E_INVALID, "bad reference index");
    return tap_one_ref(m, s, ref_index, acc_out, NULL, NULL, NULL, 0, NULL, NULL);
}

int oslam_vote_hits(oslam_model *m, oslam_scene *s, size_t ref_index, uint32_t *numbers_out, uint32_t *theta_out,
                    uint32_t *idx_out, size_t cap, size_t *n_out, uint32_t *keep_out)
{
    if (!n_out) return fail(OSLAM_E_INVALID, "NULL argument");
    *n_out = 0;
    return tap_one_ref(m, s, ref_index, NULL, numbers_out, theta_out, idx_out, cap, n_out, keep_out);
}

static int materialise_last(oslam_model *m)
{
    int rc = OSLAM_OK;
    const size_t n = m->n_last;
    if (!m->last_on_device) return OSLAM_OK;
    if (hipSetDevice(m->dev) != hipSuccess) return fail(OSLAM_E_DEVICE, "hipSetDevice failed");
    m->last_cells = (oslam_cell *)malloc(sizeof(oslam_cell) * (n ? n : 1));
    m->last_poses = (float *)malloc(sizeof(float) * 16 * (n ? n : 1));
    if (!m->last_cells || !m->last_poses) { oslam_drop_last(m); return fail(OSLAM_E_NOMEM, "host allocation failed"); }
    HIPCHK(hipMemcpy(m->last_cells, m->d_pose_cells, sizeof(oslam_cell) * n, hipMemcpyDeviceToHost));
    HIPCHK(hipMemcpy(m->last_poses, m->d_pose_T, sizeof(float) * 16 * n, hipMemcpyDeviceToHost));
    m->last_on_device = 0;
done:
    return rc;
}

int oslam_last_result(oslam_model *m, oslam_scene *s, float *trans_out, float *rots_out, float *vote_counts_out,
                      size_t cap, size_t *n_out, uint32_t *max_idx_out)
{
    int rc;
    size_t n;
    float T[16], *tr = NULL, *ro = NULL, *sc = NULL;
    uint32_t best = 0;
    if (!n_out) return fail(OSLAM_E_INVALID, "NULL argument");
    *n_out = 0;
    rc = oslam_check_pair(m, s);
    if (rc != OSLAM_OK) return rc;
    if (materialise_last(m) != OSLAM_OK) return OSLAM_E_DEVICE;
    n = m->n_last;
    if (max_idx_out) *max_idx_out = 0;
    if (n == 0) return OSLAM_OK;
    tr = (float *)calloc(3 * n, sizeof(float));
    ro = (float *)calloc(4 * n, sizeof(float));
    sc = (float *)calloc(n, sizeof(float));
    if (!tr || !ro || !sc) { rc = fail(OSLAM_E_NOMEM, "host allocation failed"); goto done; }
    rc = oslam_pose_stage_ex(m->last_cells, n, m->c.h_xyz, m->c.h_nrm, (size_t)m->c.n, s->c.h_xyz, s->c.h_nrm, (size_t)s->c.n,
                             m->d_dist, m->params.cpu_clustering, m->params.use_l1_norm, m->params.use_averaged_clusters,
                             m->weights, T, NULL, tr, ro, sc, &best);
    if (rc != OSLAM_OK) { rc = fail(rc, "pose stage failed"); goto done; }
    if (n > cap) n = cap;
    if (trans_out) memcpy(trans_out, tr, sizeof(float) * 3 * n);
    if (rots_out) memcpy(rots_out, ro, sizeof(float) * 4 * n);
    if (vote_counts_out) memcpy(vote_counts_out, sc, sizeof(float) * n);
    if (max_idx_out) *max_idx_out = best;
    *n_out = n;
done:
    free(tr);
    free(ro);
    free(sc);
    return rc;
}

int oslam_last_cells(oslam_model *m, oslam_cell *cells_out, float *poses_out, size_t cap, size_t *n_out)
{
    size_t n;
    if (!m || !n_out) return fail(OSLAM_E_INVALID, "NULL argument");
    if ((cells_out || poses_out) && materialise_last(m) != OSLAM_OK) return OSLAM_E_DEVICE;
    n = m->n_last < cap ? m->n_last : cap;
    if (cells_out) memcpy(cells_out, m->last_cells, sizeof(oslam_cell) * n);
    if (poses_out) memcpy(poses_out, m->last_poses, sizeof(float) * 16 * n);
    *n_out = m->n_last;
    return OSLAM_OK;
}

static uint64_t sm64(uint64_t *s)
{
    uint64_t z = (*s += 0x9e3779b97f4a7c15ull);
    z = (z ^ (z >> 30)) * 0xbf58476d1ce4e5b9ull;
    z = (z ^ (z >> 27)) * 0x94d049bb133111ebull;
    return z ^ (z >> 31);
}

int oslam_selftest_math(size_t n, uint64_t seed, uint64_t *mismatches)
// ... 64 lines not shown
```

objective-slam_amd/csrc/oslam_vote.c:

```c
#include <pthread.h>
#include <stdio.h>

#include "oslam_internal.h"
#include "oslam_vote_plan.h"

int oslam_check_pair(const oslam_model *m, const oslam_scene *s)
{
    if (!m || !s) return fail(OSLAM_E_INVALID, "NULL handle");
    if (m->unusable) return fail(OSLAM_E_INVALID, "this model lost its key tables with its database: it can only be destroyed");
    if (m->dev != s->dev) return fail(OSLAM_E_INVALID, "model and scene live on different devices");
    if (s->d_dist != 0.0f && m->d_dist != s->d_dist) return fail(OSLAM_E_INVALID, "scene d_dist differs from the model's (ppf.cu:64-67)");
    return OSLAM_OK;
}

#define MAX_DEVICES 64
#define MAX_BATCH_EVENTS 64
#define N_EVENTS (4 + 3 * MAX_BATCH_EVENTS)
#define SLOT_BYTES (sizeof(oslamk_pay) * 2 + sizeof(oslamk_run) + sizeof(uint32_t))

enum { HOST_NONE, HOST_PINNED, HOST_MALLOC };
typedef struct pool_buf {
    void *d, *h;
    int host;
    size_t cap;
// ... 145 lines not shown
    return OSLAM_OK;
}

static void carve_scratch(oslamk_vote_args *a, const scratch_pool *p, size_t slots)
{
    char *b = (char *)p->b[BUF_HITS].d;
    a->redo = (uint32_t *)p->b[BUF_REDO].d;
    a->hit_pay = (oslamk_pay *)b;
    b += slots * sizeof(oslamk_pay);
    a->hit_sorted = (oslamk_pay *)b;
    b += slots * sizeof(oslamk_pay);
    a->runs = (oslamk_run *)b;
    b += slots * sizeof(oslamk_run);
    a->hit_key = (uint32_t *)b;
}

int oslam_pool_read_hits(const scratch_pool *p, uint32_t *numbers_out, uint32_t *theta_out, uint32_t *idx_out, size_t cap,
                         size_t *n_out, uint32_t *keep_out)
{
    int rc = OSLAM_OK;
    oslamk_vote_args a;
    oslamk_pay *pay = NULL;
    uint32_t n = 0;
    size_t i, m;
    *n_out = 0;
    if (keep_out) *keep_out = ((const uint32_t *)p->b[BUF_COUNTS].h)[0];
    if (p->plan.nb < 1) return OSLAM_OK;
    carve_scratch(&a, p, p->plan.b[0].slots);
    HIPCHK(hipMemcpy(&n, (const uint32_t *)p->b[BUF_COUNTS].d + p->b[BUF_COUNTS].cap, sizeof n, hipMemcpyDeviceToHost));
    *n_out = n;
    m = n < cap ? n : cap;
    if (!m) return OSLAM_OK;
    pay = (oslamk_pay *)malloc(sizeof *pay * m);
    if (!pay) return fail(OSLAM_E_NOMEM, "host allocation failed");
    HIPCHK(hipMemcpy(pay, a.hit_sorted, sizeof *pay * m, hipMemcpyDeviceToHost));
    if (numbers_out) {
        HIPCHK(hipMemcpy(numbers_out, a.hit_key, sizeof(uint32_t) * m, hipMemcpyDeviceToHost));
        for (i = 0; i < m; i++) numbers_out[i] &= 0x7fffffffu;
    }
    for (i = 0; i < m; i++) {
        if (theta_out) theta_out[i] = pay[i].theta_t22;
        if (idx_out) idx_out[i] = pay[i].idx;
    }
done:
    free(pay);
    return rc;
}

#define REF_ORDER_CLASSES 1024
void oslam_ref_order(const uint32_t *keep, size_t n, uint32_t *order)
{
    uint32_t start[REF_ORDER_CLASSES + 1], top = 0;
    size_t i;
    int c;
    for (i = 0; i < n; i++) if (keep[i] > top) top = keep[i];
    if (top == 0) top = 1;
    memset(start, 0, sizeof start);
    for (i = 0; i < n; i++) start[1 + (REF_ORDER_CLASSES - 1) - (int)((uint64_t)keep[i] * (REF_ORDER_CLASSES - 1) / top)]++;
    for (c = 0; c < REF_ORDER_CLASSES; c++) start[c + 1] += start[c];
    for (i = 0; i < n; i++) order[start[(REF_ORDER_CLASSES - 1) - (int)((uint64_t)keep[i] * (REF_ORDER_CLASSES - 1) / top)]++] = (uint32_t)i;
}

typedef struct vote_pass {
    scratch_pool *pool;
    oslam_model *const *ms;
    int nm, n_ref;
    hipStream_t st;
    oslamk_vote_args a;
    uint32_t *d_keep, *d_hitc, *d_runc, *d_off, *h_keep, *h_off;
    size_t limit;
    size_t widest;
    size_t redo_stride;
    int ordered;
    int one_grid;
} vote_pass;

static void member_args(oslamk_vote_args *a, const oslam_model *m)
{
    a->table.uinfo = m->table.uinfo;
    a->table.n_slices = m->table.n_slices;
    a->table.slots = m->table.slots;
    a->table.cap = m->table.cap;
    a->ent = m->ent;
    a->thresh = m->params.vote_count_threshold;
    a->counters = m->d_counters;
    a->out = m->d_out;
    a->out_cap = m->out_cap;
    a->mode = (m->params.vote_mode == OSLAM_VOTE_FAST) ? 1 : 0;
}

static void pass_open(vote_pass *v, scratch_pool *pool, oslam_model *const *ms, int nm, const oslam_scene *s,
                      const uint32_t *d_ref_idx, const float *d_tsg, int n_ref, uint32_t fixed_gmax, uint32_t *acc_dump)
{
    int j;
    memset(v, 0, sizeof *v);
    v->pool = pool;
    v->ms = ms;
    v->nm = nm;
    v->n_ref = n_ref;
    v->st = (hipStream_t)oslam_stream();
    v->limit = scratch_limit(ms[0]);
    v->widest = 1;
    for (j = 0; j < nm; j++) if ((size_t)ms[j]->table.n_slices > v->widest) v->widest = (size_t)ms[j]->table.n_slices;
    v->ordered = (ms[0]->params.vote_order == 0 || ms[0]->params.vote_order == 3) && !acc_dump && n_ref > 1;
    v->one_grid = nm > 1 && n_ref > 0 && !acc_dump && ((size_t)n_ref + 7) / 8 * 8 * v->widest <= 2048;
    for (j = 1; j < nm && v->one_grid; j++)
        if ((ms[j]->params.vote_mode == OSLAM_VOTE_FAST) != (ms[0]->params.vote_mode == OSLAM_VOTE_FAST)) v->one_grid = 0;
    v->a.scene = s->c.k;
    v->a.order = s->order;
    v->a.ref_idx = d_ref_idx;
    v->a.tsg = d_tsg;
    v->a.n_ref = n_ref;
    v->a.d_dist = ms[0]->d_dist;
    v->a.inv_d_dist = ms[0]->inv_d_dist;
    v->a.table = ms[0]->table;
    v->a.fixed_gmax = fixed_gmax;
    v->a.acc_dump = acc_dump;
    v->a.dump_ref = acc_dump ? 0 : -1;
    member_args(&v->a, ms[0]);
}

static int pass_reserve(vote_pass *v)
{
    scratch_pool *pool = v->pool;
    const size_t n = (size_t)(v->n_ref > 0 ? v->n_ref : 1), nm = (size_t)v->nm;
    size_t need, cap;
    int rc = oslam_pool_reserve_counts(pool, n);
    if (rc != OSLAM_OK) return rc;
    need = v->redo_stride = (n + 7) / 8 * 8 * v->widest;
    if (nm > 1) need *= nm;
    cap = need + need / 4;
    rc = pool_buf_grow(&pool->b[BUF_REDO], need, cap, sizeof(uint32_t) * cap, 0);
    if (rc != OSLAM_OK) return rc;
    if (v->ordered) {
        cap = n + n / 4 + 64;
        rc = pool_buf_grow(&pool->b[BUF_ORDER], n, cap, sizeof(uint32_t) * cap, sizeof(uint32_t) * cap);
        if (rc != OSLAM_OK) return rc;
    }
    if (v->one_grid) {
        cap = nm + nm / 2 + 8;
        rc = pool_buf_grow(&pool->b[BUF_VARGS], nm, cap, sizeof(oslamk_vote_args) * cap, sizeof(oslamk_vote_args) * cap);
        if (rc != OSLAM_OK) return rc;
    }
    cap = pool->b[BUF_COUNTS].cap;
    v->d_keep = (uint32_t *)pool->b[BUF_COUNTS].d;
    v->d_hitc = v->d_keep + cap;
    v->d_runc = v->d_hitc + cap;
    v->d_off = v->d_runc + cap;
    v->h_keep = (uint32_t *)pool->b[BUF_COUNTS].h;
    v->h_off = v->h_keep + cap;
    return OSLAM_OK;
}

static int pass_demand(vote_pass *v, oslam_vote_times *t)
{
    int rc = OSLAM_OK, i;
    hipEvent_t *ev = v->pool->ev;
    float k0 = 0.0f;
    uint64_t sum = 0;
    if (v->n_ref <= 0) return OSLAM_OK;
    HIPCHK(hipMemsetAsync(v->d_keep, 0, sizeof(uint32_t) * (size_t)v->n_ref, v->st));
    v->a.first_ref = 0;
    v->a.n_launch = v->n_ref;
    v->a.keep_count = v->d_keep;
    KCHK(oslamk_scene_count(&v->a, oslam_stream()));
    HIPCHK(hipEventRecord(ev[2], v->st));
// ... 10 lines not shown
}

static int pass_plan(vote_pass *v)
{
    oslam_vote_plan *plan = &v->pool->plan;
    int rc = OSLAM_OK;
    if (oslam_vote_plan_build(plan, v->h_keep, v->n_ref, v->limit / SLOT_BYTES, v->h_off) != 0)
        return fail(OSLAM_E_NOMEM, "host allocation failed");
    rc = pool_reserve_slots(v->pool, plan->max_slots, v->limit);
    if (rc != OSLAM_OK) return rc;
    if (plan->n_off) HIPCHK(hipMemcpyAsync(v->d_off, v->h_off, sizeof(uint32_t) * plan->n_off, hipMemcpyHostToDevice, v->st));
    v->one_grid = v->one_grid && oslam_vote_plan_is_one_batch(plan);
done:
    return rc;
}

static int pass_batch(vote_pass *v, int nb)
{
    scratch_pool *pool = v->pool;
    const oslam_vote_batch *b = &pool->plan.b[nb];
    oslamk_vote_args *a = &v->a, *d_vargs = (oslamk_vote_args *)pool->b[BUF_VARGS].d, *h_vargs = (oslamk_vote_args *)pool->b[BUF_VARGS].h;
    hipEvent_t *ev = nb < MAX_BATCH_EVENTS ? pool->ev + 4 + 3 * nb : NULL;
    int rc = OSLAM_OK, j;
    a->first_ref = b->first;
    a->n_launch = b->n;
    a->keep_count = NULL;
    a->hit_off = v->d_off + b->off_at;
    a->hit_count = v->d_hitc;
    a->run_count = v->d_runc;
    carve_scratch(a, pool, b->slots);
    HIPCHK(hipMemsetAsync(v->d_hitc, 0, sizeof(uint32_t) * (size_t)b->n, v->st));
    if (ev) HIPCHK(hipEventRecord(ev[0], v->st));
    KCHK(oslamk_scene_hits(a, oslam_stream()));
    KCHK(oslamk_sort_hits(a, oslam_stream()));
    if (ev) HIPCHK(hipEventRecord(ev[1], v->st));
    a->ref_order = NULL;
    if (v->ordered) {
        uint32_t *d_order = (uint32_t *)pool->b[BUF_ORDER].d + b->first, *h_order = (uint32_t *)pool->b[BUF_ORDER].h + b->first;
        oslam_ref_order(v->h_keep + b->first, (size_t)b->n, h_order);
        HIPCHK(hipMemcpyAsync(d_order, h_order, sizeof(uint32_t) * (size_t)b->n, hipMemcpyHostToDevice, v->st));
        a->ref_order = d_order;
    }
    for (j = 0; j < v->nm; j++) {
        member_args(a, v->ms[j]);
        if (v->one_grid) {
            a->redo = (uint32_t *)pool->b[BUF_REDO].d + (size_t)j * v->redo_stride;
            h_vargs[j] = *a;
            continue;
        }
        KCHK(oslamk_vote(a, oslam_stream()));
        HIPCHK(hipMemsetAsync(&v->ms[j]->d_counters->redo_count, 0, sizeof(uint32_t), v->st));
    }
    if (v->one_grid) {
        HIPCHK(hipMemcpyAsync(d_vargs, h_vargs, sizeof(oslamk_vote_args) * (size_t)v->nm, hipMemcpyHostToDevice, v->st));
        KCHK(oslamk_vote_group(d_vargs, h_vargs, v->nm, oslam_stream()));
    }
    if (ev) HIPCHK(hipEventRecord(ev[2], v->st));
done:
    return rc;
}

static int pass_collect(vote_pass *v, oslamk_counters *cnt, oslam_vote_times *t)
{
    scratch_pool *pool = v->pool;
    const oslamk_vote_args *h_vargs = (const oslamk_vote_args *)pool->b[BUF_VARGS].h;
    hipEvent_t *ev = pool->ev;
    int rc = OSLAM_OK, i, j, again = 0;
    HIPCHK(hipEventRecord(ev[1], v->st));
    for (j = 0; j < v->nm; j++) HIPCHK(hipMemcpyAsync(&cnt[j], v->ms[j]->d_counters, sizeof *cnt, hipMemcpyDeviceToHost, v->st));
    HIPCHK(hipStreamSynchronize(v->st));
    for (j = 0; j < v->nm && v->one_grid; j++)
        if (cnt[j].redo_count) {
            KCHK(oslamk_vote_wide(&h_vargs[j], oslam_stream()));
            HIPCHK(hipMemcpyAsync(&cnt[j], v->ms[j]->d_counters, sizeof *cnt, hipMemcpyDeviceToHost, v->st));
            again = 1;
        }
    if (again) HIPCHK(hipStreamSynchronize(v->st));
    for (j = 0; j < v->nm; j++)
        if (cnt[j].list_overflow)
            return fail(OSLAM_E_DEVICE, cnt[j].list_overflow & 1u
                            ? "a hit list overflowed: the counting pass and the hit pass disagreed on the pairs within reach"
                            : cnt[j].list_overflow & 2u ? "near-edge search: a hit's key number lies outside the model's bucket records"
                            : cnt[j].list_overflow & 4u ? "near-edge search: a bucket lies outside the model's entry arrays"
                                                        : "near-edge search: a directory place lies outside its bucket segment");
    if (!t) return OSLAM_OK;
    HIPCHK(hipEventElapsedTime(&t->ms, ev[0], ev[1]));
    for (i = 0; i < pool->plan.nb && i < MAX_BATCH_EVENTS; i++) {
        float k = 0.0f, vk = 0.0f;
        HIPCHK(hipEventElapsedTime(&k, ev[4 + 3 * i], ev[4 + 3 * i + 1]));
        HIPCHK(hipEventElapsedTime(&vk, ev[4 + 3 * i + 1], ev[4 + 3 * i + 2]));
        t->ms_key_kernel += k;
        t->ms_vote_kernel += vk;
    }
    t->launches += (uint32_t)pool->plan.nb;
done:
    return rc;
}

int oslam_run_votes_group(scratch_pool *pool, oslam_model *const *ms, int nm, oslam_scene *s, const uint32_t *d_ref_idx,
                          const float *d_tsg, int n_ref, uint32_t fixed_gmax, uint32_t *acc_dump, oslamk_counters *cnt,
                          oslam_vote_times *t)
{
    vote_pass v;
    int rc = OSLAM_OK, j, nb;
    pass_open(&v, pool, ms, nm, s, d_ref_idx, d_tsg, n_ref, fixed_gmax, acc_dump);
    rc = pass_reserve(&v);
    if (rc != OSLAM_OK) return rc;
    for (j = 0; j < nm; j++) HIPCHK(hipMemsetAsync(ms[j]->d_counters, 0, sizeof(oslamk_counters), v.st));
    HIPCHK(hipEventRecord(pool->ev[0], v.st));
    rc = pass_demand(&v, t);
    if (rc == OSLAM_OK) rc = pass_plan(&v);
    for (nb = 0; rc == OSLAM_OK && nb < pool->plan.nb; nb++) rc = pass_batch(&v, nb);
    if (rc == OSLAM_OK) rc = pass_collect(&v, cnt, t);
done:
    return rc;
}

static int run_votes(scratch_pool *pool, oslam_model *m, oslam_scene *s, uint32_t fixed_gmax, oslamk_counters *cnt,
                     oslam_vote_times *t)
{
    const int rc = oslam_run_votes_group(pool, &m, 1, s, s->d_ref_idx, s->d_tsg, s->n_ref, fixed_gmax, NULL, cnt, t);
    if (rc == OSLAM_OK && fixed_gmax) cnt->gmax = fixed_gmax;
    return rc;
}

int oslam_grow_records(oslam_model *m, uint64_t need)
{
    oslamk_cell *d_new = NULL;
    oslam_cell *h_new;
    if (need > ((uint64_t)1 << 28)) return fail(OSLAM_E_LIMIT, "more than 2^28 accumulator peaks above the threshold");
    if (hipMalloc((void **)&d_new, sizeof(oslamk_cell) * need) != hipSuccess) {
        (void)hipGetLastError();
        return fail(OSLAM_E_NOMEM, "no device memory for the accumulator peaks");
    }
    h_new = (oslam_cell *)malloc(sizeof(oslam_cell) * need);
    if (!h_new) { (void)hipFree(d_new); return fail(OSLAM_E_NOMEM, "host allocation failed"); }
    (void)hipFree(m->d_out);
    free(m->h_out);
    m->d_out = d_new;
    m->h_out = h_new;
    m->out_cap = (uint32_t)need;
    m->n_local = 0;
    return OSLAM_OK;
}

void oslam_vote_stats(oslam_stats *st, const scratch_pool *pool, const oslam_model *m, const oslam_scene *s,
                      const oslamk_counters *cnt, const oslam_vote_times *t)
{
    st->num_scene_ppfs = (uint64_t)s->n_ref * (uint64_t)(s->c.n - 1);
    st->num_hits = cnt->hits;
    st->num_votes = cnt->votes;
    st->num_unique_votes = cnt->nonzero_cells;
    st->num_model_keys = m->num_model_keys;
    st->max_count = cnt->gmax;
    st->num_emitted = cnt->out_count;
    st->ms_vote = t->ms;
    st->ms_vote_kernel = t->ms_vote_kernel;
    st->ms_key_kernel = t->ms_key_kernel;
    st->vote_launches = t->launches;
    st->num_pairs_probed = t->probed;
    st->num_entries_streamed = cnt->entries;
    st->num_items = cnt->items;
    st->wide_workgroups = cnt->redo_total;
    st->scratch_bytes = pool->b[BUF_HITS].cap;
}

int oslam_vote_records(scratch_pool *pool, oslam_model *m, oslam_scene *s, oslamk_counters *cnt, size_t *n_cells,
// ... 76 lines not shown
```

objective-slam_amd/csrc/oslam_vote_body.inc:

```
#ifndef OSLAM_VOTE_BODY_INC
#define OSLAM_VOTE_BODY_INC

#define WAVE 64
#ifndef VOTE_THREADS
#define VOTE_THREADS 1024
#endif
#ifndef ACC_STRIDE
#define ACC_STRIDE 31
#endif
#define ACC_CELLS (OSLAMK_ROWS * ACC_STRIDE)
#define ACC_REAL_CELLS (1023 * ACC_STRIDE)

static __device__ const uint32_t k_alpha_thr[32] = {PC_ALPHA_THR_FLAT};

__device__ __forceinline__ uint32_t wave_max_u32(uint32_t v)
{
    for (int o = 32; o > 0; o >>= 1) {
        uint32_t w = __shfl_xor(v, o, WAVE);
        v = v > w ? v : w;
    }
    return v;
}
__device__ __forceinline__ uint32_t wave_sum_u32(uint32_t v)
{
    for (int o = 32; o > 0; o >>= 1) v += __shfl_xor(v, o, WAVE);
    return v;
}
__device__ __forceinline__ unsigned long long wave_sum_u64(unsigned long long v)
{
    for (int o = 32; o > 0; o >>= 1) v += __shfl_xor(v, o, WAVE);
    return v;
}

__device__ __forceinline__ float readlane_f(float v, int l)
{
    return __builtin_bit_cast(float, __builtin_amdgcn_readlane(__builtin_bit_cast(int, v), l));
}
__device__ __forceinline__ uint32_t readlane_u(uint32_t v, int l)
{
    return (uint32_t)__builtin_amdgcn_readlane((int)v, l);
}
__device__ __forceinline__ void vote_product(uint32_t tm8, uint32_t &bin, uint32_t &pos)
{
    const unsigned long long p = (unsigned long long)tm8 * 30ull;
    bin = (uint32_t)(p >> 32);
    pos = (uint32_t)p;
    asm("" : "+v"(bin));
}
__device__ __forceinline__ uint32_t uni_u32(uint32_t v) { return (uint32_t)__builtin_amdgcn_readfirstlane((int)v); }
__device__ __forceinline__ unsigned long long uni_u64(unsigned long long v)
{
    return ((unsigned long long)uni_u32((uint32_t)(v >> 32)) << 32) | uni_u32((uint32_t)v);
}

#define ACC_TRASH_WORDS 96

struct SlowCtx {
    const uint32_t *pw;
    const oslamk_uv *puv;
    const oslamk_pay *hits;
    const float *px, *py, *pz;
    const float *rows;
    uint32_t inc_lo, inc_hi;
    uint32_t dropped;
};

#define PM_FN(n) n##_cold
#define PM_KU(bits) ({ uint32_t pinned_; asm volatile("v_mov_b32 %0, %1" : "=v"(pinned_) : "i"(bits)); pinned_; })
#define PM_KF(bits) __builtin_bit_cast(float, PM_KU(bits))
#undef PM_HD
#define PM_HD __device__ static inline
#include "ppf_math_atan.inc"
#undef PM_FN
#undef PM_KU
#undef PM_KF
__device__ __forceinline__ unsigned alpha_bin_reeval(float uy, float uz, float vy, float vz, const uint32_t *tbl)
{
    const unsigned b = pc_alpha_bin_table_main(uy, uz, vy, vz, tbl);
    return b != PC_ALPHA_OUTSIDE ? b : pc_alpha_bin_exact_cold(uy, uz, vy, vz);
}

typedef __attribute__((address_space(3))) uint32_t lds_u32;
typedef __attribute__((address_space(3))) unsigned long long lds_u64;
typedef __attribute__((address_space(3))) SlowCtx lds_ctx;

#define SLOW_CAP 96
#define SLOW_VERIFY 0x80000000u
#define SLOW_HIT_BITS 28

__device__ __forceinline__ void slow_queue_flush(lds_ctx *sc, lds_u32 *acc, lds_u32 *tbl, lds_u64 *q, uint32_t n, int lane)
{
    const uint32_t *t = (const uint32_t *)tbl;
    for (uint32_t base = 0; base < n; base += WAVE) {
        if (base + lane < n) {
            const unsigned long long it = q[base + lane];
            const uint32_t entry = (uint32_t)it & ~SLOW_VERIFY, hi = (uint32_t)(it >> 32);
            const bool cast = ((uint32_t)it & SLOW_VERIFY) != 0u;
            const oslamk_pay hp = sc->hits[hi & ((1u << SLOW_HIT_BITS) - 1u)];
            const uint32_t i = hp.idx;
            const float x = sc->px[i], y = sc->py[i], z = sc->pz[i];
            const float vy = pc_row_dot(sc->rows, x, y, z);
            const float vz = pc_row_dot(sc->rows + 4, x, y, z);
#pragma nounroll
            for (uint32_t which = cast ? hi >> SLOW_HIT_BITS : 1u, j = 0; which; which >>= 1, j++) {
                if (!(which & 1u)) continue;
                const uint32_t ew = sc->pw[entry + j];
                const uint32_t mr = ew & PC_ROW10_MASK;
                const uint32_t inc = (ew >> PC_ROW_HALF_BIT) & 1u ? sc->inc_hi : sc->inc_lo;
                const float2 uv = *reinterpret_cast<const float2 *>(&sc->puv[entry + j]);
                const unsigned bin = alpha_bin_reeval(uv.x, uv.y, vy, vz, t);
                if (!cast) {
                    if (bin < OSLAMK_NBIN) atomicAdd((uint32_t *)&acc[mr * ACC_STRIDE + bin], inc);
                    else atomicAdd((uint32_t *)&sc->dropped, 1u);
                } else {
                    uint32_t qbin, pos;
                    vote_product(pc_vote_base_t32(hp.theta_t22) - ew, qbin, pos);
                    if (bin != qbin) {
                        atomicSub((uint32_t *)&acc[mr * ACC_STRIDE + qbin], inc);
                        if (bin < OSLAMK_NBIN) atomicAdd((uint32_t *)&acc[mr * ACC_STRIDE + bin], inc);
                        else atomicAdd((uint32_t *)&sc->dropped, 1u);
                    }
                }
            }
        }
    }
}

__device__ __forceinline__ uint32_t slow_push(lds_ctx *sc, lds_u32 *acc, lds_u32 *tbl, lds_u64 *q, uint32_t n,
                                              unsigned long long mask, uint32_t entry, uint32_t hit, int lane)
{
    if (n > SLOW_CAP - WAVE) {
        slow_queue_flush(sc, acc, tbl, q, n, lane);
        n = 0;
    }
    if ((mask >> lane) & 1ull)
        q[n + (uint32_t)__popcll(mask & ((1ull << lane) - 1ull))] = (unsigned long long)entry | ((unsigned long long)hit << 32);
    return n + (uint32_t)__popcll(mask);
}

struct VoteStep {
    uint32_t e0;
    uint32_t nl;
    uint32_t h0;
    uint32_t ne, nh;
    uint32_t R;
// ... 78 lines not shown
                         "v_mul_hi_u32 %[t1], %[t1], 30\n\t"
                         "v_mul_hi_u32 %[t2], %[t2], 30\n\t"
                         "v_mul_hi_u32 %[t3], %[t3], 30\n\t"
                         VOTE_ADDR("%[t0]", "%[r0]") VOTE_ADDR("%[t1]", "%[r1]") VOTE_ADDR("%[t2]", "%[r2]") VOTE_ADDR("%[t3]", "%[r3]") VOTE_ATOMICS
                         "s_cbranch_scc1 .Lvote_hit_%=\n\t"
                         "s_mov_b64 exec, %[sv]"
                         : [sv] "=&s"(saved), [c] "=&s"(c), [i] "+s"(i), [t0] "=&v"(t0), [t1] "=&v"(t1), [t2] "=&v"(t2), [t3] "=&v"(t3)
                         : [live] "s"(live), [csmv] "v"(csmv), [i1] "s"(d.i1), [w0] "v"(wa[0]), [w1] "v"(wa[1]), [w2] "v"(wa[2]),
                           [w3] "v"(wa[3]), [r0] "v"(rowb[0]), [r1] "v"(rowb[1]), [r2] "v"(rowb[2]), [r3] "v"(rowb[3]), [n0] "v"(inc[0]),
                           [n1] "v"(inc[1]), [n2] "v"(inc[2]), [n3] "v"(inc[3])
                         : "scc", "memory");
#undef VOTE_ATOMICS
#undef VOTE_ADDR
        }
    }
};

#define VOTE_QCAP 1024
#ifndef VOTE_BLOCK
#define VOTE_BLOCK 16
#endif
#ifndef VOTE_TAIL
#define VOTE_TAIL VOTE_BLOCK
#endif
#ifndef VOTE_TAIL_RUNS
#define VOTE_TAIL_RUNS 0
#endif
#ifndef VOTE_GIANT
#define VOTE_GIANT 16
#endif
#ifndef VOTE_WIDE_DIRECT
#define VOTE_WIDE_DIRECT (1ull << 27)
#endif
#ifndef VOTE_GROUP
#define VOTE_GROUP 8
#endif
#define RUN_SLOT_MASK ((1u << OSLAMK_RUN_SHIFT) - 1u)

template <int MODE, int PASS>
__device__ __forceinline__ void vote_body(const oslamk_vote_args &a, const uint32_t wg)
{
    __shared__ __attribute__((aligned(16))) uint32_t acc[ACC_CELLS + ACC_TRASH_WORDS];
    __shared__ uint32_t s_wave[VOTE_THREADS / WAVE];
    __shared__ uint32_t s_wave2[VOTE_THREADS / WAVE];
    __shared__ unsigned long long s_tot[2];
    __shared__ unsigned long long s_sum[VOTE_THREADS / WAVE];
    __shared__ uint32_t s_redo;
    __shared__ uint32_t s_g, s_lmax, s_base, s_qn, s_next;
    __shared__ uint32_t s_tbl[32];
    __shared__ uint32_t s_q[VOTE_QCAP];
    __shared__ SlowCtx s_ctx;
    __shared__ unsigned long long s_slow[MODE == 0 ? (VOTE_THREADS / WAVE) * SLOW_CAP : 1];

    typedef VoteRegs<MODE> VR;
    const int tid = threadIdx.x, lane = tid & (WAVE - 1), wid = tid / WAVE;
    const uint32_t nsl = (uint32_t)a.table.n_slices;
    const uint32_t xg = wg & 7u, xi = wg >> 3;
    const uint32_t ref_pos = (xi / nsl) * 8u + xg;
    const int slice = (int)(xi % nsl);
    if (ref_pos >= (uint32_t)a.n_launch) return;
    const int ref_local = (int)(a.ref_order ? uni_u32(a.ref_order[ref_pos]) : ref_pos);
    if ((uint32_t)ref_local >= (uint32_t)a.n_launch) return;
    const int ref_ord = a.first_ref + ref_local;
    const uint32_t r = a.ref_idx[ref_ord];
    const uint32_t n_runs = a.run_count[ref_local];
    const size_t off = a.hit_off[ref_local];
    const oslamk_pay *hits = a.hit_sorted + off;
    const oslamk_run *runs = a.runs + off;
    const oslamk_uinfo *uinfo = a.table.uinfo + (size_t)slice * a.table.uinfo_stride;
    const uint32_t e_first = uni_u32(a.table.slots[(size_t)slice * a.table.cap].start);
    const uint32_t *e4 = a.ent.e4 + e_first;
    const uint32_t m_base = (uint32_t)slice * OSLAMK_SLICE;
    if (tid == 0) {
        s_ctx.pw = a.ent.pw;
        s_ctx.puv = a.ent.puv;
        s_ctx.hits = hits;
        s_ctx.px = a.scene.px;
        s_ctx.py = a.scene.py;
        s_ctx.pz = a.scene.pz;
        s_ctx.rows = a.tsg + 8 * (size_t)ref_ord;
        s_ctx.inc_lo = PASS == 2 ? 0u : 1u;
        s_ctx.inc_hi = PASS == 0 ? 0x10000u : PASS == 2 ? 1u : 0u;
        s_ctx.dropped = 0;
    }
    const SlowCtx *sc = &s_ctx;

    for (int c = tid; c < ACC_CELLS / 4; c += VOTE_THREADS) reinterpret_cast<uint4 *>(acc)[c] = make_uint4(0, 0, 0, 0);
    if (tid < 32) s_tbl[tid] = k_alpha_thr[tid];

    unsigned long long *sq = s_slow + (MODE == 0 ? wid * SLOW_CAP : 0);
    uint32_t sq_n = 0;
#ifdef VOTE_PROF
    const long long pt0 = clock64();
#endif

    uint32_t T = VOTE_GIANT;
    for (bool first = true;; first = false) {
        if (tid == 0) {
            s_qn = 0;
            s_next = 0;
            if (first) s_tot[0] = s_tot[1] = 0;
        }
        __syncthreads();
        for (uint32_t k0 = 0; k0 < n_runs; k0 += VOTE_THREADS) {
            const uint32_t k = k0 + (uint32_t)tid;
            bool giant = false;
            unsigned long long lv = 0, le = 0;
            if (k < n_runs) {
                const oslamk_run rr = runs[k];
                const uint32_t lf = uinfo[rr.slot_r & RUN_SLOT_MASK].len;
                const uint32_t ln = lf & 0x7fffffffu, R = (rr.slot_r >> OSLAMK_RUN_SHIFT) + 1u;
                lv = (unsigned long long)ln * R;
                le = ((unsigned long long)(ln != 0u) << 40) + ln;
                giant = ((ln + 255u) >> 8) * R > T && !(MODE == 0 && ((lf | rr.first) >> 31));
            }
            if (first) {
                lv = wave_sum_u64(lv);
                le = wave_sum_u64(le);
                if (lane == 0 && le) {
                    atomicAdd(&s_tot[0], lv);
                    atomicAdd(&s_tot[1], le);
                }
            }
            const unsigned long long gm = __ballot(giant);
            if (gm) {
                uint32_t base = 0;
                if (lane == 0) base = atomicAdd(&s_qn, (uint32_t)__popcll(gm));
                base = readlane_u(base, 0);
                const uint32_t p = base + (uint32_t)__popcll(gm & ((1ull << lane) - 1ull));
                if (giant && p < VOTE_QCAP) s_q[p] = k;
            }
        }
        __syncthreads();
        if (s_qn <= VOTE_QCAP) break;
        T *= 2;
        __syncthreads();
    }
    const uint32_t n_q = uni_u32(s_qn);
    T = uni_u32(T);
    if (PASS == 0 && s_tot[0] > VOTE_WIDE_DIRECT) {
        if (tid == 0) {
            a.redo[atomicAdd(&a.counters->redo_count, 1u)] = wg;
            atomicAdd(&a.counters->redo_total, 1u);
        }
        return;
    }
#ifdef VOTE_PROF
    const long long ptA = clock64();
#endif

    const uint32_t pass = PASS;
    const uint32_t inc_lo = PASS == 2 ? 0u : 1u, inc_hi = PASS == 0 ? 0x10000u : PASS == 2 ? 1u : 0u;
    {
        uint2 B_ru = make_uint2(0, 0), B_inf = make_uint2(0, 0);
        auto bperm = [&](uint32_t from_lane, uint32_t v) -> uint32_t {
            return (uint32_t)__builtin_amdgcn_ds_bpermute((int)(from_lane << 2), (int)v);
        };
        auto step_at = [&](uint32_t ve0, uint32_t vh0, uint32_t vmisc, int l) -> VoteStep {
            VoteStep d;
            const uint32_t misc = readlane_u(vmisc, l);
            d.e0 = readlane_u(ve0, l);
            d.h0 = readlane_u(vh0, l);
            d.ne = d.e0 + (misc >> 20) * 16u;
            d.nh = d.h0 + (misc & 63u) * 8u + 8u;
            d.R = (misc & 63u) + 1u;
            d.i0 = (misc >> 6) & 127u;
            d.i1 = (misc >> 13) & 127u;
            d.nl = misc >> 20;
            d.valid = true;
            return d;
        };
        auto split_of = [&](uint32_t R, bool split) -> uint32_t { return !split ? 0u : R > 32u ? 2u : R > 16u ? 1u : 0u; };
        auto vote_set = [&](bool take, bool split, uint32_t u0, uint32_t stride) {
            uint32_t excl, incl;
            {
                const uint32_t R = (B_ru.x >> OSLAMK_RUN_SHIFT) + 1u;
                const uint32_t nu = take ? (((B_inf.y & 0x7fffffffu) + 255u) >> 8) << split_of(R, split) : 0u;
                incl = nu;
                for (int o = 1; o < WAVE; o <<= 1) {
                    const uint32_t up = __shfl_up(incl, o, WAVE);
                    if (lane >= o) incl += up;
                }
                excl = incl - nu;
            }
            const uint32_t total = readlane_u(incl, WAVE - 1);
            for (uint32_t ub = u0; ub < total; ub += stride * WAVE) {
                const uint32_t u = ub + stride * (uint32_t)lane;
                const bool act = u < total;
                uint32_t lo = 0;
    #pragma unroll
                for (uint32_t s2 = WAVE / 2; s2 > 0; s2 >>= 1) lo += bperm(lo + s2 - 1u, incl) <= u ? s2 : 0u;
                lo = lo < (uint32_t)WAVE - 1u ? lo : (uint32_t)WAVE - 1u;
                const uint32_t st = bperm(lo, B_inf.x), ln = bperm(lo, B_inf.y) & 0x7fffffffu, h0 = bperm(lo, B_ru.y) & 0x7fffffffu;
                const uint32_t R = (bperm(lo, B_ru.x) >> OSLAMK_RUN_SHIFT) + 1u, lg = split_of(R, split);
                const uint32_t local = u - bperm(lo, excl);
                const uint32_t c = local >> lg, hs = local & ((1u << lg) - 1u), per = (R + (1u << lg) - 1u) >> lg;
                const uint32_t i0 = hs * per, i1 = i0 + per < R ? i0 + per : R;
                const uint32_t left = ln - (c << 8), nl = left < 256u ? (left + 3u) >> 2 : 64u;
                const uint32_t w_e0 = act ? (st - e_first + (c << 8)) * 4u : 0u, w_h0 = act ? h0 * 8u : 0u,
                               w_misc = act ? (R - 1u) | (i0 << 6) | (i1 << 13) | (nl << 20) : 0u;
                const uint32_t rest = (total - ub + stride - 1u) / stride, n_w = rest < (uint32_t)WAVE ? rest : (uint32_t)WAVE;
                for (uint32_t g0 = 0; g0 < n_w; g0 += VOTE_GROUP) {
                    VR regs[VOTE_GROUP];
                    VoteStep ds[VOTE_GROUP];
    #pragma unroll
                    for (int g = 0; g < VOTE_GROUP; g++) {
                        ds[g] = step_at(w_e0, w_h0, w_misc, (int)g0 + g);
                        regs[g].load(e4, hits, ds[g], lane);
                    }
                    asm volatile("" ::: "memory");
    #pragma unroll
                    for (int g = 0; g < VOTE_GROUP; g++) regs[g].vote(acc, ds[g], lane, inc_lo, inc_hi);
                }
            }
        };
        const uint32_t *skeys = a.hit_key + off;
        const uint32_t n_hits = a.hit_count[ref_local] < (uint32_t)(a.hit_off[ref_local + 1] - off) ? a.hit_count[ref_local]
                                                                                                   : (uint32_t)(a.hit_off[ref_local + 1] - off);
        const uint32_t n_cq = (n_hits + WAVE - 1u) / WAVE;
        uint32_t cq = uni_u32((uint32_t)wid);
#ifdef VOTE_PROF
        long long prof_corr = 0;
#endif
        auto correct_pass = [&]() {
#ifdef VOTE_PROF
            const long long pc0 = clock64();
#endif
            const uint32_t *pw = a.ent.pw;
            const uint16_t *pdir = a.ent.pdir;
            const uint32_t hit = cq * WAVE + (uint32_t)lane;
            cq += VOTE_THREADS / WAVE;
            const bool in = hit < n_hits;
            const uint32_t kw = skeys[in ? hit : 0u];
            const bool key_ok = (kw & RUN_SLOT_MASK) < a.table.uinfo_stride;
            const oslamk_uinfo ui = uinfo[key_ok ? kw & RUN_SLOT_MASK : 0u];
            uint32_t ln = in && key_ok && !((kw | ui.len) >> 31) ? ui.len : 0u;
            const bool bucket_ok = ln == 0u || (ui.start <= a.ent.n_real && ln <= a.ent.n_real - ui.start);
            if (!bucket_ok) ln = 0;
            if (__ballot((in && !key_ok) || !bucket_ok)) {
                if (in && !key_ok) atomicOr(&a.counters->list_overflow, 2u);
                if (!bucket_ok) atomicOr(&a.counters->list_overflow, 4u);
            }
            const uint32_t A = pc_vote_base_t32(hits[in ? hit : 0u].theta_t22) * 30u - (PC_T24_EDGE - 1u), B = A + (PC_T24_EDGE - 1u);
            for (uint32_t seg = 0; __ballot(seg < ln); seg += OSLAMK_PSEG) {
                const uint32_t n = seg < ln ? (ln - seg < OSLAMK_PSEG ? ln - seg : OSLAMK_PSEG) : 0u;
                const uint32_t sbase = n ? ui.start + seg : 0u, K = OSLAMK_PDIR_CELLS(n);
                const uint32_t cA = __umulhi(A, K), cB = __umulhi(B, K);
                const uint32_t d0 = n ? pdir[((size_t)sbase << OSLAMK_PDIR_SHIFT) + cA] : 0u, d1 = n ? pdir[((size_t)sbase << OSLAMK_PDIR_SHIFT) + cB + 1u] : 0u;
                uint32_t cnt = K == 1u ? n : B < A ? n - d0 + d1 : d1 - d0;
#ifdef VOTE_DIAG_NOCAND
                cnt = 0;
#endif
                if (d0 > n || d1 > n || cnt > 2u * n) {
                    atomicOr(&a.counters->list_overflow, 8u);
                    cnt = 0;
                }
                uint32_t incl = cnt;
                for (int o = 1; o < WAVE; o <<= 1) {
                    const uint32_t up = __shfl_up(incl, o, WAVE);
                    if (lane >= o) incl += up;
                }
                const uint32_t excl = incl - cnt, total = readlane_u(incl, WAVE - 1);
                const uint32_t hit0 = hit - (uint32_t)lane;
                for (uint32_t base = 0; base < total; base += 4u * WAVE) {
                    uint32_t kk[4], own[4], w[4];
                    bool inl[4];
    #pragma unroll
                    for (int u = 0; u < 4; u++) {
                        const uint32_t f = base + (uint32_t)u * WAVE + (uint32_t)lane;
                        inl[u] = f < total;
                        kk[u] = own[u] = w[u] = 0;
                        if (base + (uint32_t)u * WAVE >= total) continue;
                        uint32_t o = 0;
    #pragma unroll
                        for (uint32_t s2 = WAVE / 2; s2 > 0; s2 >>= 1) o += bperm(o + s2 - 1u, incl) <= f ? s2 : 0u;
                        o = o < (uint32_t)WAVE - 1u ? o : (uint32_t)WAVE - 1u;
                        const uint32_t no = bperm(o, n), d0o = bperm(o, d0), exo = bperm(o, excl), sbo = bperm(o, sbase);
                        uint32_t k = d0o + (f - exo);
                        k = k >= no ? k - no : k;
                        k = k < no ? k : 0u;
                        own[u] = o;
                        kk[u] = inl[u] ? sbo + k : 0u;
                        w[u] = pw[kk[u]];
                    }
    #pragma unroll
                    for (int u = 0; u < 4; u++) {
                        if (base + (uint32_t)u * WAVE >= total) continue;
                        const uint32_t Ao = bperm(own[u], A);
                        const bool near = inl[u] && w[u] * 30u - Ao < PC_T24_EDGE;
                        const unsigned long long nm = __ballot(near);
                        if (nm) sq_n = slow_push((lds_ctx *)sc, (lds_u32 *)acc, (lds_u32 *)s_tbl, (lds_u64 *)sq, sq_n, nm, kk[u] | SLOW_VERIFY, (hit0 + own[u]) | (1u << SLOW_HIT_BITS), lane);
                    }
                }
            }
#ifdef VOTE_PROF
            prof_corr += clock64() - pc0;
#endif
        };
        auto marked = [&](const uint2 &ru, const uint2 &inf) -> bool { return MODE == 0 && ((inf.y | ru.y) >> 31); };

        {
            const uint32_t tail_runs = n_runs < VOTE_TAIL_RUNS ? n_runs : VOTE_TAIL_RUNS;
            const uint32_t n_big = (n_runs - tail_runs) / VOTE_BLOCK;
            const uint32_t n_blocks = n_big + (n_runs - n_big * VOTE_BLOCK + VOTE_TAIL - 1) / VOTE_TAIL;
            auto block_first = [&](uint32_t b) -> uint32_t { return b < n_big ? b * VOTE_BLOCK : n_big * VOTE_BLOCK + (b - n_big) * VOTE_TAIL; };
            auto block_len = [&](uint32_t b) -> uint32_t { return b < n_big ? (uint32_t)VOTE_BLOCK : (uint32_t)VOTE_TAIL; };
            const uint32_t my_slot = (uint32_t)lane / VOTE_BLOCK, k_in = (uint32_t)lane % VOTE_BLOCK;
            auto grab = [&]() -> uint32_t {
                uint32_t b = 0;
                if (lane == 0) b = atomicAdd(&s_next, 1u);
                return uni_u32(readlane_u(b, 0));
            };
            auto fetch_runs = [&](uint32_t b, uint32_t slot) {
                if (my_slot == slot) {
                    const uint32_t k = block_first(b) + k_in;
                    B_ru = make_uint2(0, 0);
                    B_inf = make_uint2(0, 0);
                    if (k_in < block_len(b) && k < n_runs) {
                        const oslamk_run rr = runs[k];
                        B_ru = make_uint2(rr.slot_r, rr.first);
                    }
                }
            };
            auto fetch_info = [&](uint32_t b, uint32_t slot) {
                if (my_slot == slot && k_in < block_len(b) && block_first(b) + k_in < n_runs) {
                    const oslamk_uinfo ui = uinfo[B_ru.x & RUN_SLOT_MASK];
                    B_inf = make_uint2(ui.start, ui.len);
                }
            };
            uint32_t cur_b = 0, nx1_b = 0, nx2_b = 0, turn = 0;
            uint32_t tw = 0;
            bool started = false;
            for (;;) {
                bool take, split;
                uint32_t u0, stride;
                if (tw < n_q) {
                    const uint32_t t = tw + (uint32_t)lane;
                    B_ru = make_uint2(0, 0);
                    B_inf = make_uint2(0, 0);
                    if (t < n_q) {
                        const oslamk_run rr = runs[s_q[t]];
                        const oslamk_uinfo ui = uinfo[rr.slot_r & RUN_SLOT_MASK];
                        B_ru = make_uint2(rr.slot_r, rr.first);
                        B_inf = make_uint2(ui.start, ui.len);
                    }
                    tw += WAVE;
                    take = t < n_q;
                    split = true;
                    u0 = uni_u32((uint32_t)wid);
                    stride = VOTE_THREADS / WAVE;
                } else {
                    if (!started) {
                        started = true;
                        cur_b = grab();
                        fetch_runs(cur_b, 0u);
                        nx1_b = grab();
                        fetch_runs(nx1_b, 1u);
                        nx2_b = grab();
                        fetch_runs(nx2_b, 2u);
                        fetch_info(cur_b, 0u);
                        fetch_info(nx1_b, 1u);
                    }
                    if (cur_b >= n_blocks) break;
                    const uint32_t ln = B_inf.y & 0x7fffffffu, R = (B_ru.x >> OSLAMK_RUN_SHIFT) + 1u;
                    take = my_slot == (turn & 3u) && ln != 0u && ((ln + 255u) >> 8) * R <= T && !marked(B_ru, B_inf);
                    split = false;
                    u0 = 0u;
                    stride = 1u;
                    cur_b = nx1_b;
                    nx1_b = nx2_b;
                    fetch_info(nx1_b, (turn + 2u) & 3u);
                    nx2_b = grab();
                    fetch_runs(nx2_b, (turn + 3u) & 3u);
                    turn++;
                }
                vote_set(take, split, u0, stride);
#ifndef VOTE_DIAG_NOCORRECT
// ... 11 lines not shown
#endif
        if (MODE == 0) {
            for (uint32_t k0 = (uint32_t)wid * WAVE; k0 < n_runs; k0 += VOTE_THREADS) {
                const uint32_t k = k0 + (uint32_t)lane;
                oslamk_run rr;
                oslamk_uinfo ui;
                rr.slot_r = rr.first = 0;
                ui.start = ui.len = 0;
                if (k < n_runs) {
                    rr = runs[k];
                    ui = uinfo[rr.slot_r & RUN_SLOT_MASK];
                }
                unsigned long long fm = __ballot((ui.len & 0x7fffffffu) != 0u && ((ui.len | rr.first) >> 31));
                while (fm) {
                    const int j = __ffsll((long long)fm) - 1;
                    fm &= fm - 1ull;
                    sq_n = forced_item((lds_ctx *)sc, (lds_u32 *)acc, (lds_u32 *)s_tbl, (lds_u64 *)sq, sq_n, readlane_u(ui.start, j),
                                       readlane_u(ui.len, j) & 0x7fffffffu, readlane_u(rr.first, j) & 0x7fffffffu,
                                       (readlane_u(rr.slot_r, j) >> OSLAMK_RUN_SHIFT) + 1u, lane);
                }
            }
            if (sq_n) slow_queue_flush((lds_ctx *)sc, (lds_u32 *)acc, (lds_u32 *)s_tbl, (lds_u64 *)sq, sq_n, lane);
        }
#ifdef VOTE_PROF
        const long long pt1 = clock64();
#endif
        asm volatile("s_waitcnt lgkmcnt(0)" ::: "memory");
        __syncthreads();
#ifdef VOTE_PROF
        const long long pt2 = clock64();
        if (lane == 0) {
            atomicAdd(&a.counters->prof[0], (unsigned long long)(ptA - pt0));
            atomicAdd(&a.counters->prof[1], (unsigned long long)(pt1 - ptA));
            atomicAdd(&a.counters->prof[2], (unsigned long long)(pt2 - pt1));
        }
#endif


        auto lower_of = [&](uint32_t w) -> uint32_t { return pass == 0 ? w & 0xffffu : pass == 1 ? w : 0u; };
        auto upper_of = [&](uint32_t w) -> uint32_t { return pass == 0 ? w >> 16 : pass == 2 ? w : 0u; };
        uint32_t lmax = 0, nz = 0;
        unsigned long long sum = 0;
#pragma unroll 2
        for (int c = tid; c < ACC_REAL_CELLS; c += VOTE_THREADS) {
            const uint32_t w = acc[c], v0 = lower_of(w), v1 = upper_of(w);
            lmax = max(lmax, max(v0, v1));
            nz += (v0 != 0) + (v1 != 0);
            sum += (unsigned long long)v0 + v1;
        }
        lmax = wave_max_u32(lmax);
        nz = wave_sum_u32(nz);
        sum = wave_sum_u64(sum);
        if (lane == 0) {
            s_wave[wid] = lmax;
            s_wave2[wid] = nz;
            s_sum[wid] = sum;
        }
        __syncthreads();
        if (tid == 0) {
            uint32_t m = 0, n = 0;
            unsigned long long tot = 0;
            for (int w = 0; w < VOTE_THREADS / WAVE; w++) {
                m = s_wave[w] > m ? s_wave[w] : m;
                n += s_wave2[w];
                tot += s_sum[w];
            }
            s_redo = pass == 0 && tot != s_tot[0] - s_ctx.dropped;
#if defined(VOTE_DIAG_NOLOOP) || defined(VOTE_DIAG_NOATOM)
            s_redo = 0;
#endif
            if (s_redo) {
                a.redo[atomicAdd(&a.counters->redo_count, 1u)] = wg;
                atomicAdd(&a.counters->redo_total, 1u);
            }
            if (!s_redo) {
                if (pass <= 1) {
                    const unsigned long long h = slice == 0 ? (unsigned long long)a.hit_count[ref_local] : 0ull;
                    if (h) atomicAdd(&a.counters->hits, h);
                    if (s_tot[0]) atomicAdd(&a.counters->votes, s_tot[0]);
                    if (s_tot[1]) {
                        atomicAdd(&a.counters->entries, s_tot[1] & 0xffffffffffull);
                        atomicAdd(&a.counters->items, s_tot[1] >> 40);
                    }
                }
                uint32_t g = a.fixed_gmax;
                if (g == 0) {
                    const uint32_t old = atomicMax(&a.counters->gmax, m);
                    g = old > m ? old : m;
                }
                if (n) atomicAdd(&a.counters->nonzero_cells, (unsigned long long)n);
                s_g = g;
                s_lmax = m;
            }
        }
        __syncthreads();
        if (s_redo) return;

        if (a.acc_dump && ref_ord == a.dump_ref) {
            uint32_t *dst = a.acc_dump + (size_t)m_base * OSLAMK_NBIN;
    #pragma unroll 2
        for (int c = tid; c < ACC_REAL_CELLS; c += VOTE_THREADS) {
                const uint32_t w = acc[c];
                const int cell = c / ACC_STRIDE * OSLAMK_NBIN + c % ACC_STRIDE;
                if (pass <= 1) dst[cell] = lower_of(w);
                if (pass != 1) dst[cell + (int)PC_ROWS_PER_HALF * OSLAMK_NBIN] = upper_of(w);
                if (ACC_STRIDE < OSLAMK_NBIN && c % ACC_STRIDE == ACC_STRIDE - 1) {
                    if (pass <= 1) dst[cell + 1] = 0;
                    if (pass != 1) dst[cell + 1 + (int)PC_ROWS_PER_HALF * OSLAMK_NBIN] = 0;
                }
            }
        }

        const float bound = a.thresh * (float)s_g;
        if ((float)s_lmax > bound) {
            uint32_t cnt = 0;
    #pragma unroll 2
        for (int c = tid; c < ACC_REAL_CELLS; c += VOTE_THREADS) {
                const uint32_t w = acc[c];
                cnt += ((float)lower_of(w) > bound) + ((float)upper_of(w) > bound);
            }
            uint32_t incl = cnt;
            for (int o = 1; o < WAVE; o <<= 1) {
                const uint32_t up = __shfl_up(incl, o, WAVE);
                if (lane >= o) incl += up;
            }
            if (lane == WAVE - 1) s_wave[wid] = incl;
            __syncthreads();
            if (tid == 0) {
                uint32_t run = 0;
                for (int w = 0; w < VOTE_THREADS / WAVE; w++) {
                    const uint32_t v = s_wave[w];
                    s_wave[w] = run;
                    run += v;
                }
                s_base = atomicAdd(&a.counters->out_count, run);
            }
            __syncthreads();
            uint32_t pos = s_base + s_wave[wid] + incl - cnt;
    #pragma unroll 2
        for (int c = tid; c < ACC_REAL_CELLS; c += VOTE_THREADS) {
                const uint32_t w = acc[c];
#pragma unroll
                for (int hf = 0; hf < 2; hf++) {
                    const uint32_t v = hf ? upper_of(w) : lower_of(w);
                    if ((float)v > bound) {
                        if (pos < a.out_cap) {
                            oslamk_cell cell;
                            const uint32_t m_r = m_base + (uint32_t)hf * PC_ROWS_PER_HALF + (uint32_t)(c / ACC_STRIDE);
                            cell.code = ((unsigned long long)r << 32) | (unsigned long long)((m_r << 6) |
                                                                         (uint32_t)(c % ACC_STRIDE));
                            cell.count = v;
                            cell.pad = 0;
                            a.out[pos] = cell;
                        }
                        pos++;
                    }
                }
            }
        }
    }
}

#endif
```

objective-slam_amd/csrc/ppf_core.h:

```cpp
#ifndef OSLAM_PPF_CORE_H
#define OSLAM_PPF_CORE_H

#include "ppf_acos_table.h"
#include "ppf_alpha_table.h"
#include "ppf_math.h"

#include <math.h>
#define PC_FMODF(x, y) fmodf((x), (y))

PM_HD uint32_t pc_quant_bits(float x, float step, float inv_step)
{
    int k;
    float q = pm_quant_down_pos(x, step, inv_step, &k);
    if (k < 0) q = x - PC_FMODF(x, step);
    if (pm_isnan(q)) return PM_NAN_BITS;
    return PM_BITS_F2U(q);
}

PM_HD int pc_pair_dist_bin(float dx, float dy, float dz, float d_dist, float inv_d_dist)
{
    int k;
    (void)pm_quant_down_pos(pm_sqrtf(dx * dx + dy * dy + dz * dz), d_dist, inv_d_dist, &k);
    return k;
}
// ... 82 lines not shown
PM_HD float pc_row_dot(const float *row, float px, float py, float pz)
{
    return row[0] * px + row[1] * py + row[2] * pz + row[3] * 1.0f;
}


#define PC_ALPHA_OUTSIDE 0xffffffffu
PM_HD unsigned pc_alpha_bin_table_main(float uy, float uz, float vy, float vz, const uint32_t *tbl)
{
    const float cx = uy * vz - uz * vy;
    const float dt = 0.0f * 0.0f + uy * vy + uz * vz;
    const uint32_t hy = PM_BITS_F2U(cx), hx = PM_BITS_F2U(dt);
    const uint32_t iy = hy & 0x7fffffffu, ix = hx & 0x7fffffffu;
    const int k = ((int32_t)iy - (int32_t)ix) >> 23;
    if ((iy - 1u) < 0x7f7fffffu && (ix - 1u) < 0x7f7fffffu && (unsigned)(k + 60) <= 120u) {
        const uint32_t qb = PM_BITS_F2U(PM_BITS_U2F(iy) / PM_BITS_U2F(ix));
        const unsigned m = (hy >> 31) | ((hx >> 31) << 1);
        const uint32_t *row = tbl + 8 * m;
        unsigned pos = (row[4] <= qb) ? 4u : 0u;
        const unsigned tiny = row[0] <= qb;
        pos += (row[pos + 2] <= qb) ? 2u : 0u;
        pos += (row[pos + 1] <= qb) ? 1u : 0u;
        pos += tiny;
        return (m == 0u) ? 15u + pos : (m == 1u) ? 15u - pos : (m == 2u) ? 30u - pos : pos;
    }
    return PC_ALPHA_OUTSIDE;
}
PM_HD unsigned pc_alpha_bin_table(float uy, float uz, float vy, float vz, const uint32_t *tbl)
{
    const unsigned b = pc_alpha_bin_table_main(uy, uz, vy, vz, tbl);
    return b != PC_ALPHA_OUTSIDE ? b : pc_alpha_bin_exact(uy, uz, vy, vz);
}

#define PC_T22_TURN 4194304u
#define PC_T24_SCALE 7680u
#define PC_T24_MARGIN 64u
#define PC_T24_EDGE (2u * PC_T24_MARGIN * PC_T24_SCALE)
#define PC_T22_FORCE 0xffffffffu
#define PC_T22_PER_RAD 667544.214430109f

PM_HD uint32_t pc_angle_t22(float y, float z)
{
    const uint32_t by = PM_BITS_F2U(y) & 0x7fffffffu, bz = PM_BITS_F2U(z) & 0x7fffffffu;
    const uint32_t e = (by > bz ? by : bz) >> 23;
    const float q = __builtin_rintf((pm_atan2f(z, y) + PM_PI_F) * PC_T22_PER_RAD);
    if (e < 87u || e > 167u || !(q >= 0.0f && q <= 4194304.0f)) return PC_T22_FORCE;
    return (uint32_t)q & (PC_T22_TURN - 1u);
}

PM_HD uint32_t pc_vote_base_t24(uint32_t theta_v_t22)
{
    return ((theta_v_t22 + PC_T22_TURN / 2u) << 2) + PC_T24_MARGIN;
}

#define PC_ROW_BITS 11
#define PC_ROW_MASK 0x7ffu
#define PC_ROW10_MASK 0x3ffu
#define PC_ROW_HALF_BIT 10
#define PC_ROW_SINK 1023u
#define PC_ROWS_PER_HALF 1023u
PM_HD uint32_t pc_theta_u21(uint32_t theta_t22) { return ((theta_t22 + 1u) >> 1) & (PC_T22_TURN / 2u - 1u); }
PM_HD uint32_t pc_entry_word(uint32_t theta_u_t22, uint32_t row11) { return (pc_theta_u21(theta_u_t22) << PC_ROW_BITS) | row11; }
PM_HD uint32_t pc_row11(uint32_t local) { return ((local / PC_ROWS_PER_HALF) << PC_ROW_HALF_BIT) | (local % PC_ROWS_PER_HALF); }
PM_HD uint32_t pc_local_of_row11(uint32_t row11) { return (row11 >> PC_ROW_HALF_BIT) * PC_ROWS_PER_HALF + (row11 & PC_ROW10_MASK); }
PM_HD uint32_t pc_vote_base_t32(uint32_t theta_v_t22) { return (pc_vote_base_t24(theta_v_t22) << 8) + 1024u; }

PM_HD unsigned pc_alpha_bin_hybrid_ex(float uy, float uz, float vy, float vz, uint32_t row, const uint32_t *tbl,
                                      int *needs_exact, double *pos_bins)
{
    const uint32_t cs = pc_angle_t22(vy, vz), am = pc_angle_t22(uy, uz);
    const uint32_t tm32 = pc_vote_base_t32(cs) - pc_entry_word(am, row);
    const uint64_t prod = (uint64_t)tm32 * 30u;
    const int slow = cs == PC_T22_FORCE || am == PC_T22_FORCE || (uint32_t)prod < PC_T24_EDGE;
    if (needs_exact) *needs_exact = slow;
    if (pos_bins) *pos_bins = (double)((((cs + PC_T22_TURN / 2u) << 2) - (pc_theta_u21(am) << 3)) & 0xffffffu) * 30.0 / 16777216.0;
    if (slow) return pc_alpha_bin_table(uy, uz, vy, vz, tbl);
    return (unsigned)(prod >> 32);
}
PM_HD unsigned pc_alpha_bin_hybrid(float uy, float uz, float vy, float vz, uint32_t row, const uint32_t *tbl)
{
    return pc_alpha_bin_hybrid_ex(uy, uz, vy, vz, row, tbl, 0, 0);
}

#define PC_FAST_BOUND 3.1e-5
PM_HD uint32_t pc_vote_base_fast_t32(uint32_t theta_v_t22) { return pc_vote_base_t32(theta_v_t22) - (PC_T24_MARGIN << 8); }
PM_HD uint32_t pc_theta_fast(uint32_t theta_t22) { return theta_t22 == PC_T22_FORCE ? 0u : theta_t22; }
PM_HD unsigned pc_alpha_bin_fast(float uy, float uz, float vy, float vz, uint32_t row)
{
    const uint32_t cs = pc_theta_fast(pc_angle_t22(vy, vz)), am = pc_theta_fast(pc_angle_t22(uy, uz));
    return (unsigned)(((uint64_t)(pc_vote_base_fast_t32(cs) - pc_entry_word(am, row)) * 30u) >> 32);
}

#endif
```

objective-slam_amd/ppf.py:

```python
import ctypes as C
import os

import numpy as np

_HERE = os.path.dirname(os.path.abspath(__file__))
LIB_PATH = os.environ.get("OSLAM_LIB", os.path.join(_HERE, "liboslam_hip.so"))
_LIB = None

OSLAM_OK, OSLAM_E_INVALID, OSLAM_E_DEVICE, OSLAM_E_NOMEM, OSLAM_E_NO_VOTES, OSLAM_E_LIMIT, OSLAM_E_PEER = range(7)
STAGE_VOTE, STAGE_SELECT, STAGE_GROW = 1, 2, 3
VOTE_EXACT, VOTE_FAST = 0, 1
COMM_ID_BYTES = 128


class OslamError(RuntimeError):
    def __init__(self, code, msg):
        super().__init__("oslam error %d: %s" % (code, msg))
        self.code = code


class Params(C.Structure):
    _fields_ = [("ref_point_df", C.c_uint), ("vote_count_threshold", C.c_float),
                ("cpu_clustering", C.c_int), ("use_l1_norm", C.c_int), ("use_averaged_clusters", C.c_int),
                ("dev", C.c_int), ("vote_mode", C.c_int), ("shard_rank", C.c_int), ("shard_world", C.c_int),
                ("max_cells", C.c_uint), ("pose_gpu_min", C.c_uint), ("no_bucket_spread", C.c_int),
                ("scratch_gib", C.c_uint), ("pose_two_sorts", C.c_int), ("vote_order", C.c_int), ("reserved", C.c_int * 1)]


class Stats(C.Structure):
    _fields_ = [("num_scene_ppfs", C.c_uint64), ("num_hits", C.c_uint64), ("num_votes", C.c_uint64),
                ("num_unique_votes", C.c_uint64), ("num_model_keys", C.c_uint64), ("num_top", C.c_uint64),
                ("max_count", C.c_uint32), ("num_emitted", C.c_uint32), ("ms_vote", C.c_float),
                ("ms_total", C.c_float), ("vote_launches", C.c_uint32), ("ms_vote_kernel", C.c_float),
                ("ms_key_kernel", C.c_float), ("wide_workgroups", C.c_uint32), ("num_pairs_probed", C.c_uint64),
                ("scratch_bytes", C.c_uint64), ("num_entries_streamed", C.c_uint64), ("num_items", C.c_uint64)]

    def asdict(self):
        return {f: getattr(self, f) for f, _ in self._fields_}


class RefineParams(C.Structure):
    _fields_ = [("max_iterations", C.c_uint), ("max_corr_dist", C.c_float), ("min_normal_dot", C.c_float),
                ("inlier_dist", C.c_float), ("min_fitness", C.c_float), ("stop_rot", C.c_float), ("stop_trans", C.c_float),
                ("reserved", C.c_int * 4)]


class RefineResult(C.Structure):
    _fields_ = [("fitness_in", C.c_float), ("fitness", C.c_float), ("rmse", C.c_float), ("inliers", C.c_uint32),
                ("correspondences", C.c_uint32), ("iterations", C.c_uint32), ("converged", C.c_int32),
                ("found", C.c_int32), ("launches", C.c_uint32), ("ms_total", C.c_float)]

    def asdict(self):
        return {f: getattr(self, f) for f, _ in self._fields_}


class VerifyParams(C.Structure):
    _fields_ = [("depth_tol", C.c_float), ("window", C.c_uint), ("min_view_fitness", C.c_float),
                ("min_coverage", C.c_float), ("min_supported", C.c_uint), ("reserved", C.c_int * 4)]


class VerifyResult(C.Structure):
    _fields_ = [("back", C.c_uint32), ("out", C.c_uint32), ("supported", C.c_uint32), ("occluded", C.c_uint32),
                ("conflict", C.c_uint32), ("unknown", C.c_uint32), ("view_fitness", C.c_float), ("coverage", C.c_float),
                ("found", C.c_int32), ("launches", C.c_uint32), ("ms_total", C.c_float)]

    def asdict(self):
        return {f: getattr(self, f) for f, _ in self._fields_}


VERIFY_BACK, VERIFY_OUT, VERIFY_SUPPORTED, VERIFY_OCCLUDED, VERIFY_CONFLICT, VERIFY_UNKNOWN = range(6)


class InstanceParams(C.Structure):
    _fields_ = [("max_instances", C.c_uint), ("min_separation", C.c_float), ("max_angle", C.c_float),
                ("min_score_ratio", C.c_float), ("keep_not_found", C.c_int), ("reserved", C.c_int * 4)]


class Instance(C.Structure):
    _fields_ = [("T", C.c_float * 16), ("T_vote", C.c_float * 16), ("score", C.c_float), ("candidate", C.c_uint32),
                ("refine", RefineResult)]

    def astuple(self):
        T = np.array(self.T, np.float32).reshape(4, 4)
        return T, {"T_vote": np.array(self.T_vote, np.float32).reshape(4, 4), "score": float(self.score),
                   "candidate": int(self.candidate), "refine": self.refine.asdict()}


MAX_INSTANCES = 64


class ArbitrateParams(C.Structure):
    _fields_ = [("depth_tol", C.c_float), ("window", C.c_uint), ("tile", C.c_uint), ("tile_spacing", C.c_float),
                ("min_tiles", C.c_uint), ("min_owned_share", C.c_float), ("reserved", C.c_int * 4)]


class ArbitrateResult(C.Structure):
    _fields_ = [("claimed", C.c_uint32), ("owned", C.c_uint32), ("share", C.c_float), ("mean_residual", C.c_float),
                ("kept", C.c_int32), ("suppressed_by", C.c_int32), ("tile", C.c_uint32), ("rounds", C.c_uint32),
                ("launches", C.c_uint32), ("ms_total", C.c_float)]

    def asdict(self):
        return {f: getattr(self, f) for f, _ in self._fields_}


class DetectParams(C.Structure):
    _fields_ = [("instances", InstanceParams), ("refine", RefineParams), ("verify", VerifyParams),
                ("arbitrate", ArbitrateParams), ("reserved", C.c_int * 4)]


# ... 352 lines not shown
    "oslam_pyramid_destroy": (_i, [_vp]),
    "oslam_pyramid_level": (_i, [_vp, _u, C.POINTER(_vp)]),
    "oslam_pyramid_egomotion": (_i, [_vp, _vp, _vp, C.POINTER(EgomotionParams), _vp, C.POINTER(EgomotionResult)]),
    "oslam_volume_track_pyramid": (_i, [_vp, _vp, _vp, C.POINTER(PyramidParams), C.POINTER(EgomotionParams), _vp,
                                        C.POINTER(EgomotionResult)]),
    "oslam_render_params_default": (_i, [C.POINTER(RenderParams)]),
    "oslam_render_create": (_i, [_vp, _vp, _sz, _vp, _i, _i, C.POINTER(RenderParams), C.POINTER(_vp), _vp]),
    "oslam_db_render": (_i, [_vp, _vp, _vp, _sz, _vp, _i, _i, C.POINTER(RenderParams), C.POINTER(_vp), _vp]),
    "oslam_render_view": (_i, [_vp, C.POINTER(_vp)]),
    "oslam_explain_params_default": (_i, [C.POINTER(ExplainParams)]),
    "oslam_explain": (_i, [_vp, _vp, _sz, _vp, C.POINTER(ExplainParams), _vp]),
    "oslam_db_explain": (_i, [_vp, _vp, _vp, C.POINTER(ExplainParams), _vp]),
    "oslam_explain_rect": (_i, [_vp, C.c_double, _vp, _vp, _i, _i, C.c_uint, _vp]),
    "oslam_explain_z": (_i, [_vp, _vp, _sz, _vp, C.POINTER(ExplainParams), _sz, _vp]),
    "oslam_explain_claims": (_i, [_vp, _vp, _sz, _vp, C.POINTER(ExplainParams), _vp, _vp, _sz, C.POINTER(C.c_uint32),
                                  C.POINTER(_sz)]),
    "oslam_render_labels": (_i, [_vp, _vp]),
    "oslam_render_destroy": (_i, [_vp]),
    "oslam_view_info": (_i, [_vp, _vp, C.POINTER(_i), C.POINTER(_i)]),
    "oslam_mask_params_default": (_i, [C.POINTER(MaskParams)]),
    "oslam_view_mask": (_i, [_vp, _vp, C.POINTER(MaskParams), C.POINTER(_vp), C.POINTER(MaskResult)]),
    "oslam_bilateral_params_default": (_i, [C.POINTER(BilateralParams)]),
    "oslam_view_bilateral": (_i, [_vp, C.POINTER(BilateralParams), C.POINTER(_vp), C.POINTER(BilateralResult)]),
    "oslam_gauss_table": (_i, [_u, C.POINTER(_f)]),
    "oslam_surface_params_default": (_i, [C.POINTER(SurfaceParams)]),
    "oslam_volume_surface": (_i, [_vp, C.POINTER(SurfaceParams), _vp, _vp, _sz, C.POINTER(_sz), C.POINTER(SurfaceResult)]),
    "oslam_scene_from_volume": (_i, [_vp, C.POINTER(SurfaceParams), _f, _f, _u, C.POINTER(Params), C.POINTER(_vp),
                                     C.POINTER(_sz)]),
    "oslam_volume_set_voxels": (_i, [_vp, _vp, _vp]),
    "oslam_volume_shift": (_i, [_vp, _vp, C.POINTER(ShiftResult)]),
    "oslam_volume_window": (_i, [_vp, _vp, _vp]),
    "oslam_volume_leaving": (_i, [_vp, _vp, C.POINTER(SurfaceParams), _vp, _vp, _sz, C.POINTER(_sz), C.POINTER(SurfaceResult)]),
    "oslam_follow_params_default": (_i, [_vp, C.POINTER(FollowParams)]),
    "oslam_volume_follow": (_i, [_vp, _vp, C.POINTER(FollowParams), _vp]),
    "oslam_world_params_of": (_i, [_vp, C.POINTER(WorldParams)]),
    "oslam_world_create": (_i, [C.POINTER(WorldParams), C.POINTER(_vp)]),
    "oslam_world_destroy": (_i, [_vp]),
    "oslam_world_clear": (_i, [_vp]),
    "oslam_world_stats_get": (_i, [_vp, C.POINTER(WorldStats)]),
    "oslam_world_put": (_i, [_vp, _vp, _vp, _sz]),
    "oslam_world_box": (_i, [_vp, _vp, _vp, _vp, _i]),
    "oslam_world_has_colour": (_i, [_vp]),
    "oslam_world_put_colour": (_i, [_vp, _vp, _vp, _vp, _sz]),
    "oslam_world_box_colour": (_i, [_vp, _vp, _vp, _vp, _vp, _i]),
    "oslam_world_colours": (_i, [_vp, _vp, C.POINTER(WorldSurfaceParams), _vp, _sz, _sz, _vp, _vp, C.POINTER(_sz)]),
    "oslam_world_surface_params_default": (_i, [C.POINTER(WorldSurfaceParams)]),
    "oslam_world_surface": (_i, [_vp, _vp, C.POINTER(WorldSurfaceParams), _vp, _vp, _vp, _sz, C.POINTER(_sz),
                                 C.POINTER(WorldSurfaceResult)]),
    "oslam_world_mesh": (_i, [_vp, _vp, C.POINTER(WorldSurfaceParams), _vp, _vp, _vp, _sz, _vp, _sz, C.POINTER(_sz),
                              C.POINTER(_sz), C.POINTER(WorldMeshResult)]),
    "oslam_world_bricks": (_i, [_vp, _vp, _sz, C.POINTER(_sz)]),
    "oslam_scene_from_world": (_i, [_vp, _vp, C.POINTER(WorldSurfaceParams), _f, _f, _u, C.POINTER(Params), C.POINTER(_vp),
                                    C.POINTER(_sz)]),
    "oslam_volume_shift_world": (_i, [_vp, _vp, _vp, C.POINTER(ReloadResult)]),
    "oslam_volume_pack": (_i, [_vp, _vp, _vp, _vp, _sz, C.POINTER(_sz)]),
    "oslam_volume_pack_colour": (_i, [_vp, _vp, _vp, _vp, _vp, _sz, C.POINTER(_sz)]),
    "oslam_mesh_params_default": (_i, [C.POINTER(MeshParams)]),
    "oslam_volume_mesh": (_i, [_vp, C.POINTER(MeshParams), _vp, _vp, _sz, _vp, _sz, C.POINTER(_sz), C.POINTER(_sz),
                               C.POINTER(MeshResult)]),
    "oslam_ply_write_mesh": (_i, [C.c_char_p, _vp, _vp, _sz, _vp, _sz, _i]),
    "oslam_mc_table_row": (_i, [_u, _vp, C.POINTER(_u)]),
    "oslam_normals_params_default": (_i, [C.POINTER(NormalsParams)]),
    "oslam_cloud_normals": (_i, [_vp, _sz, _sz, C.POINTER(NormalsParams), _i, _vp, _vp, _vp, C.POINTER(NormalsResult)]),
    "oslam_cloud_normal_moments": (_i, [_vp, _sz, _sz, C.POINTER(NormalsParams), _i, _vp]),
    "oslam_mesh_normals": (_i, [_vp, _sz, _sz, _vp, _sz, _vp, _vp]),
    "oslam_ply_read_mesh": (_i, [C.c_char_p, C.POINTER(_vp), C.POINTER(_vp), C.POINTER(_vp), C.POINTER(_sz), C.POINTER(_sz)]),
    "oslam_view_set_colour": (_i, [_vp, _vp, _sz, _vp]),
    "oslam_view_colour": (_i, [_vp, _vp]),
    "oslam_view_has_colour": (_i, [_vp]),
    "oslam_colour_params_default": (_i, [C.POINTER(ColourParams)]),
    "oslam_volume_colour_enable": (_i, [_vp, C.POINTER(ColourParams)]),
    "oslam_volume_colour_words": (_i, [_vp, _vp]),
    "oslam_volume_set_colour_words": (_i, [_vp, _vp]),
    "oslam_volume_integrate_colour": (_i, [_vp, _vp, _vp, _vp, C.POINTER(IntegrateResult), C.POINTER(C.c_uint32)]),
    "oslam_volume_colours": (_i, [_vp, _vp, _sz, _sz, _vp, _vp, C.POINTER(_sz)]),
    "oslam_volume_paint_view": (_i, [_vp, _vp, _vp, C.POINTER(C.c_uint32)]),
    "oslam_ply_write_colour": (_i, [C.c_char_p, _vp, _vp, _vp, _sz, _i]),
    "oslam_ply_write_mesh_colour": (_i, [C.c_char_p, _vp, _vp, _vp, _sz, _vp, _sz, _i]),
    "oslam_scene_keys": (_i, [_vp, _sz, _vp]),
    "oslam_model_keys": (_i, [_vp, _sz, _vp]),
    "oslam_model_bucket": (_i, [_vp, C.c_uint32, _vp, _sz, C.POINTER(_sz)]),
    "oslam_model_bucket_words": (_i, [_vp, C.c_uint32, _i, _vp, _sz, C.POINTER(_sz)]),
    "oslam_vote_accumulator": (_i, [_vp, _vp, _sz, _vp]),
    "oslam_vote_hits": (_i, [_vp, _vp, _sz, _vp, _vp, _vp, _sz, C.POINTER(_sz), C.POINTER(C.c_uint32)]),
    "oslam_model_key_numbers": (_i, [_vp, _vp, _vp, _vp, _sz, C.POINTER(_sz)]),
    "oslam_vote_ref_order": (_i, [_vp, _sz, _vp]),
    "oslam_last_cells": (_i, [_vp, _vp, _vp, _sz, C.POINTER(_sz)]),
    "oslam_set_stream": (_i, [_vp]),
    "oslam_last_error": (C.c_char_p, []),
    "oslam_set_host_threads": (_i, [_i]),
    "oslam_selftest_math": (_i, [_sz, C.c_uint64, C.POINTER(C.c_uint64)]),
}


def lib():
    global _LIB
    if _LIB is None:
        if not os.path.exists(LIB_PATH):
            raise OslamError(OSLAM_E_DEVICE, "%s not built: run `python -c 'import __graft_entry__ as g; g.build()'` "
                                             "(there is no CPU fallback)" % LIB_PATH)
        L = C.CDLL(LIB_PATH)
        for name, (res, args) in _SIGNATURES.items():
            fn = getattr(L, name)
            fn.restype = res
            fn.argtypes = args
        _LIB = L
    return _LIB


def _check(rc):
    if rc != OSLAM_OK:
        raise OslamError(rc, lib().oslam_last_error().decode("utf-8", "replace"))


def _p(a):
    return a.ctypes.data_as(C.c_void_p)


DEFAULT_OVERRIDES = {}


def default_params(**kw):
    p = Params()
    _check(lib().oslam_params_default(C.byref(p)))
    for k, v in {**DEFAULT_OVERRIDES, **kw}.items():
        if not hasattr(p, k):
            raise TypeError("unknown parameter %r" % k)
        setattr(p, k, v)
    return p


def vote_ref_order(keep):
    keep = np.ascontiguousarray(keep, np.uint32)
    out = np.zeros(len(keep), np.uint32)
    _check(lib().oslam_vote_ref_order(_p(keep), len(keep), _p(out)))
    return out


def default_refine_params(**kw):
    p = RefineParams()
    _check(lib().oslam_refine_params_default(C.byref(p)))
    for k, v in kw.items():
        if not hasattr(p, k) or k == "reserved":
            raise TypeError("unknown refine parameter %r" % k)
        setattr(p, k, v)
    return p


def default_verify_params(**kw):
    p = VerifyParams()
    _check(lib().oslam_verify_params_default(C.byref(p)))
    for k, v in kw.items():
        if not hasattr(p, k) or k == "reserved":
            raise TypeError("unknown verify parameter %r" % k)
        setattr(p, k, v)
    return p


def default_instance_params(**kw):
    p = InstanceParams()
    _check(lib().oslam_instance_params_default(C.byref(p)))
    for k, v in kw.items():
        if not hasattr(p, k) or k == "reserved":
            raise TypeError("unknown instance parameter %r" % k)
        setattr(p, k, v)
    return p
# ... 430 lines not shown
        self.params = params if params is not None else default_params()
        self.d_dist, self.df = float(d_dist), int(ref_point_downsample_factor)
        sp = _world_surface_params(min_weight, anchor, dev)
        n = C.c_size_t(0)
        _check(lib().oslam_scene_from_world(world._h, vol._h if vol is not None else None, C.byref(sp), float(leaf), self.d_dist,
                                            self.df, C.byref(self.params), C.byref(self._h), C.byref(n)))
        self.n = n.value
        return self

    def numPoints(self):
        return self.n

    def getHashKeys(self, ref_index):
        out = np.zeros(self.n, np.uint32)
        _check(lib().oslam_scene_keys(self._h, int(ref_index), _p(out)))
        return out

    def close(self):
        if self._h:
            lib().oslam_scene_destroy(self._h)
            self._h = C.c_void_p(0)

    def __del__(self):
        try:
            self.close()
        except Exception:
            pass


class Model:

    def __init__(self, points, normals=None, d_dist=None, vote_count_threshold=0.4, cpu_clustering=False,
                 use_l1_norm=False, use_averaged_clusters=False, params=None):
        if d_dist is None:
            raise TypeError("d_dist is required")
        self._h = C.c_void_p(0)
        xyz, nrm, n, stride, keep = _cloud_args(points, normals)
        self.params = params if params is not None else default_params()
        self.params.vote_count_threshold = float(vote_count_threshold)
        self.params.cpu_clustering = int(cpu_clustering)
        self.params.use_l1_norm = int(use_l1_norm)
        self.params.use_averaged_clusters = int(use_averaged_clusters)
        self.d_dist = float(d_dist)
        self.n = n
        self.best_T = None
        self.stats = None
        _check(lib().oslam_model_create(xyz, nrm, n, stride, self.d_dist, C.byref(self.params), C.byref(self._h)))

    @classmethod
    def from_mesh(cls, points, triangles, d_dist=None, **kw):
        pts = np.ascontiguousarray(points, np.float32)
        nrm, valid = mesh_normals(pts, triangles)
        return cls(pts[valid], nrm[valid], d_dist=d_dist, **kw)

    def numPoints(self):
        return self.n

    def save(self, path):
        _check(lib().oslam_model_save(self._h, os.fsencode(path)))

    @classmethod
    def load(cls, path, params=None):
        self = cls.__new__(cls)
        self._h = C.c_void_p(0)
        self.params = params if params is not None else default_params()
        self.best_T = None
        self.stats = None
        _check(lib().oslam_model_load(os.fsencode(path), C.byref(self.params) if params is not None else None,
                                      C.byref(self._h)))
        n, d = C.c_size_t(0), C.c_float(0)
        _check(lib().oslam_model_info(self._h, C.byref(n), C.byref(d), None))
        self.n, self.d_dist = n.value, d.value
        return self

    def table_bytes(self):
        b = C.c_uint64(0)
        _check(lib().oslam_model_info(self._h, None, None, C.byref(b)))
        return int(b.value)

    def SetModelPointVoteWeights(self, weights):
        w = np.ascontiguousarray(weights, np.float32)
        _check(lib().oslam_model_set_point_weights(self._h, _p(w), len(w)))

    def prepare(self, scene):
        _check(lib().oslam_align_prepare(self._h, scene._h))

    def ppf_lookup(self, scene, allow_no_votes=False):
        T = np.zeros(16, np.float32)
        st = Stats()
        rc = lib().oslam_align(self._h, scene._h, _p(T), C.byref(st))
        if not (allow_no_votes and rc == OSLAM_E_NO_VOTES):
            _check(rc)
        self.best_T = T.reshape(4, 4)
        self.stats = st.asdict()
        return self.best_T

    def refine(self, scene, T=None, params=None):
        if T is None:
            T = self.best_T
        if T is None:
            raise ValueError("no pose: run ppf_lookup first or pass T")
        Ti = _pose16(T)
        To = np.zeros(16, np.float32)
        r = RefineResult()
        p = params if params is not None else default_refine_params()
        _check(lib().oslam_refine(self._h, scene._h, _p(Ti), C.byref(p), _p(To), C.byref(r)))
        return To.reshape(4, 4), r.asdict()

    def verify(self, view, T, params=None):
        r = VerifyResult()
        p = params if params is not None else default_verify_params()
        _check(lib().oslam_verify(self._h, view._h, _p(_pose16(T)), C.byref(p), C.byref(r)))
        return r.asdict()

    def find_instances(self, scene, refine=True, params=None, refine_params=None):
        ip, rp = _instance_args(refine, params, refine_params)
        cap = int(ip.max_instances)
        out = (Instance * max(cap, 1))()
        n = C.c_size_t(0)
        st = Stats()
        rc = lib().oslam_align_instances(self._h, scene._h, C.byref(ip), C.byref(rp) if rp is not None else None, out,
                                         cap, C.byref(n), C.byref(st))
        if rc != OSLAM_E_NO_VOTES:
            _check(rc)
        self.stats = st.asdict()
        return [out[k].astuple() for k in range(n.value)]

    def align_local(self, scene, cap=None):
        n = C.c_size_t(0)
        lmax = C.c_uint32(0)
        st = Stats()
        if cap is None:
            _check(lib().oslam_align_local(self._h, scene._h, None, 0, C.byref(n), C.byref(lmax), C.byref(st)))
            self.stats = st.asdict()
            return int(n.value), int(lmax.value)
        cells = np.zeros(cap, CELL_DTYPE)
        _check(lib().oslam_align_local(self._h, scene._h, _p(cells), cap, C.byref(n), C.byref(lmax), C.byref(st)))
        self.stats = st.asdict()
        return cells[: n.value].copy(), int(lmax.value)

    def local_peaks(self, global_max):
        n = C.c_size_t(0)
        rc = lib().oslam_local_peaks(self._h, int(global_max), None, 0, C.byref(n))
        if rc not in (OSLAM_OK, OSLAM_E_LIMIT):
            _check(rc)
        cells = np.zeros(max(n.value, 1), CELL_DTYPE)
        _check(lib().oslam_local_peaks(self._h, int(global_max), _p(cells), len(cells), C.byref(n)))
        return cells[: n.value].copy()

    def align_multi(self, scene, comm, allow_no_votes=False):
        T = np.zeros(16, np.float32)
        st = Stats()
        rc = lib().oslam_align_multi(self._h, scene._h, comm._h, _p(T), C.byref(st))
        if not (allow_no_votes and rc == OSLAM_E_NO_VOTES):
            _check(rc)
        self.best_T = T.reshape(4, 4)
        self.stats = st.asdict()
        return self.best_T

    def align_finish(self, scene, cells, global_max, allow_no_votes=False):
        cells = np.ascontiguousarray(cells, CELL_DTYPE)
        T = np.zeros(16, np.float32)
        st = Stats()
        rc = lib().oslam_align_finish(self._h, scene._h, _p(cells), len(cells), int(global_max), _p(T), C.byref(st))
        if not (allow_no_votes and rc == OSLAM_E_NO_VOTES):
            _check(rc)
        self.best_T = T.reshape(4, 4)
        if self.stats is not None:
            self.stats["num_top"], self.stats["max_count"] = st.num_top, st.max_count
        return self.best_T

    def last_cells(self):
        n = C.c_size_t(0)
        _check(lib().oslam_last_cells(self._h, None, None, 0, C.byref(n)))
        cells = np.zeros(n.value, CELL_DTYPE)
        poses = np.zeros((n.value, 16), np.float32)
        if n.value:
            _check(lib().oslam_last_cells(self._h, _p(cells), _p(poses), n.value, C.byref(n)))
        return cells, poses

    @property
    def transformations(self):
        return self.last_cells()[1]

    def last_result(self, scene):
        n = C.c_size_t(0)
        _check(lib().oslam_last_cells(self._h, None, None, 0, C.byref(n)))
        k = max(n.value, 1)
        tr, ro, sc = np.zeros((k, 3), np.float32), np.zeros((k, 4), np.float32), np.zeros(k, np.float32)
        best = C.c_uint32(0)
        _check(lib().oslam_last_result(self._h, scene._h, _p(tr), _p(ro), _p(sc), k, C.byref(n), C.byref(best)))
        return tr[: n.value], ro[: n.value], sc[: n.value], int(best.value)

    def getHashKeys(self, ref_index):
        out = np.zeros(self.n, np.uint32)
        _check(lib().oslam_model_keys(self._h, int(ref_index), _p(out)))
        return out

    def bucket(self, key, cap=1 << 20):
        out = np.zeros(cap, np.uint32)
        n = C.c_size_t(0)
        _check(lib().oslam_model_bucket(self._h, int(key), _p(out), cap, C.byref(n)))
        return out[: min(n.value, cap)].copy(), n.value

    def bucket_words(self, key, slice_index=0, cap=1 << 20):
        out = np.zeros(cap, np.uint32)
        n = C.c_size_t(0)
        _check(lib().oslam_model_bucket_words(self._h, int(key), int(slice_index), _p(out), cap, C.byref(n)))
        return out[: min(n.value, cap)].copy()

    def key_numbers(self):
        n = C.c_size_t(0)
        _check(lib().oslam_model_key_numbers(self._h, None, None, None, 0, C.byref(n)))
        keys, nums, w = np.zeros(n.value, np.uint32), np.zeros(n.value, np.uint32), np.zeros(n.value, np.uint64)
        if n.value:
            _check(lib().oslam_model_key_numbers(self._h, _p(keys), _p(nums), _p(w), n.value, C.byref(n)))
        return keys, nums, w

    def vote_accumulator(self, scene, ref_index):
        acc = np.zeros((self.n, 32), np.uint32)
        _check(lib().oslam_vote_accumulator(self._h, scene._h, int(ref_index), _p(acc)))
        return acc

    def vote_hits(self, scene, ref_index):
        n, keep = C.c_size_t(0), C.c_uint32(0)
        _check(lib().oslam_vote_hits(self._h, scene._h, int(ref_index), None, None, None, 0, C.byref(n), C.byref(keep)))
        num, th, idx = (np.zeros(n.value, np.uint32) for _ in range(3))
        if n.value:
            _check(lib().oslam_vote_hits(self._h, scene._h, int(ref_index), _p(num), _p(th), _p(idx), n.value, C.byref(n), C.byref(keep)))
        return num, th, idx, int(keep.value)

    def close(self):
        if getattr(self, "_db", None) is not None:
            self._db.close()
        if self._h:
            lib().oslam_model_destroy(self._h)
            self._h = C.c_void_p(0)

    def __del__(self):
        try:
# ... 1005 lines not shown
```

Measured before the change: 26.14 billion scene PPFs/s.

## Add per-segment occupancy bitmap to skip empty near-edge directory searches

```diff
diff --git a/include/oslam.h b/include/oslam.h
--- a/include/oslam.h
+++ b/include/oslam.h
@@ -35,7 +35,7 @@
     unsigned scratch_gib;
     int pose_two_sorts;
     int vote_order;
-    int reserved[1];
+    int no_edge_filter;
 } oslam_params;
 
 typedef struct oslam_stats {
@@ -765,6 +765,7 @@
                             size_t *n_out);
 int oslam_vote_ref_order(const uint32_t *keep, size_t n, uint32_t *order_out);
 int oslam_vote_accumulator(oslam_model *m, oslam_scene *s, size_t ref_index, uint32_t *acc_out);
+int oslam_vote_edge_counts(const oslam_model *m, uint64_t *edge_votes, uint64_t *edge_candidates);
 int oslam_vote_hits(oslam_model *m, oslam_scene *s, size_t ref_index, uint32_t *numbers_out, uint32_t *theta_out,
                     uint32_t *idx_out, size_t cap, size_t *n_out, uint32_t *keep_out);
 int oslam_last_cells(oslam_model *m, oslam_cell *cells_out, float *poses_out, size_t cap,
diff --git a/objective-slam_amd/csrc/oslam_host.c b/objective-slam_amd/csrc/oslam_host.c
--- a/objective-slam_amd/csrc/oslam_host.c
+++ b/objective-slam_amd/csrc/oslam_host.c
@@ -46,6 +46,7 @@
     p->no_bucket_spread = 0;
     p->scratch_gib = 0;
     p->vote_order = 0;
+    p->no_edge_filter = 0;
     return OSLAM_OK;
 }
 
diff --git a/objective-slam_amd/csrc/oslam_internal.h b/objective-slam_amd/csrc/oslam_internal.h
--- a/objective-slam_amd/csrc/oslam_internal.h
+++ b/objective-slam_amd/csrc/oslam_internal.h
@@ -29,6 +29,7 @@
     oslamk_entries ent;
     uint32_t n_entries;
     uint64_t num_model_keys;
+    uint64_t edge_votes, edge_candidates;
     float *weights;
     oslamk_counters *d_counters;
     oslamk_cell *d_out;
diff --git a/objective-slam_amd/csrc/oslam_kernels.h b/objective-slam_amd/csrc/oslam_kernels.h
--- a/objective-slam_amd/csrc/oslam_kernels.h
+++ b/objective-slam_amd/csrc/oslam_kernels.h
@@ -30,12 +30,17 @@
     uint32_t *pw;
     oslamk_uv *puv;
     uint16_t *pdir;
+    uint32_t *pocc;
     uint32_t n_real;
 } oslamk_entries;
 #define OSLAMK_PSEG 4096
 #ifndef OSLAMK_PDIR_SHIFT
 #define OSLAMK_PDIR_SHIFT 0
 #endif
+#ifndef OSLAMK_POCC_SHIFT
+#define OSLAMK_POCC_SHIFT 3
+#endif
+#define OSLAMK_POCC_WORDS(entries) ((size_t)(entries) >> (5 - OSLAMK_POCC_SHIFT))
 #define OSLAMK_PDIR_CELLS_RAW(m) ((m) <= 1u ? 1u : 1u << (31 - __builtin_clz((m) - 1u)))
 #define OSLAMK_PDIR_CELLS(n) (OSLAMK_PDIR_CELLS_RAW((n) << OSLAMK_PDIR_SHIFT) > 4096u ? 4096u : OSLAMK_PDIR_CELLS_RAW((n) << OSLAMK_PDIR_SHIFT))
 
@@ -91,6 +96,8 @@
     unsigned long long prof[4];
     uint32_t list_overflow;
     uint32_t pad_;
+    unsigned long long edge_votes;
+    unsigned long long edge_candidates;
 } oslamk_counters;
 
 typedef struct oslamk_cell {
@@ -114,6 +121,7 @@
 
 int oslamk_bucket_spread(oslamk_table t, oslamk_entries ent, void *stream);
 int oslamk_bucket_psort(oslamk_table t, oslamk_entries ent, void *stream);
+int oslamk_bucket_occupancy(oslamk_table t, oslamk_entries ent, void *stream);
 
 typedef struct oslamk_pay {
     uint32_t theta_t22;
diff --git a/objective-slam_amd/csrc/oslam_kernels.hip b/objective-slam_amd/csrc/oslam_kernels.hip
--- a/objective-slam_amd/csrc/oslam_kernels.hip
+++ b/objective-slam_amd/csrc/oslam_kernels.hip
@@ -352,6 +352,33 @@
             }
             ent.pdir[(base << OSLAMK_PDIR_SHIFT) + k] = (uint16_t)lo;
         }
+        __syncthreads();
+    }
+}
+
+static_assert((1ull << 32) / PC_OCC_MAX_CELLS > PC_T24_EDGE && (1ull << 32) / 4096u > PC_T24_EDGE,
+              "a cell of the directory or of the occupancy bits must not be narrower than the margin window");
+static_assert(OSLAMK_POCC_SHIFT >= 3 && OSLAMK_POCC_SHIFT <= 5 && (OSLAMK_PSEG << OSLAMK_POCC_SHIFT) >= PC_OCC_MAX_CELLS,
+              "a bucket's bits start on a word, and a full segment owns the largest number of cells");
+__global__ __launch_bounds__(SPREAD_THREADS) void k_bucket_occupancy(oslamk_table t, oslamk_entries ent)
+{
+    __shared__ uint32_t s_occ[PC_OCC_MAX_CELLS / 32];
+    const oslamk_slot sl = t.slots[blockIdx.x];
+    if (sl.key == 0 || sl.len == 0) return;
+    if (sl.start > ent.n_real || sl.len > ent.n_real - sl.start) return;
+    const int tid = threadIdx.x;
+    for (uint32_t seg = 0; seg < sl.len; seg += OSLAMK_PSEG) {
+        const uint32_t n = sl.len - seg < OSLAMK_PSEG ? sl.len - seg : OSLAMK_PSEG;
+        const size_t base = (size_t)sl.start + seg;
+        const uint32_t Kf = pc_occ_cells(n << OSLAMK_POCC_SHIFT);
+        for (uint32_t k = tid; k < Kf / 32u; k += SPREAD_THREADS) s_occ[k] = 0u;
+        __syncthreads();
+        for (uint32_t i = tid; i < n; i += SPREAD_THREADS) {
+            const uint32_t c = pc_occ_cell(ent.pw[base + i] * 30u, Kf);
+            atomicOr(&s_occ[c >> 5], 1u << (c & 31u));
+        }
+        __syncthreads();
+        for (uint32_t k = tid; k < Kf / 32u; k += SPREAD_THREADS) ent.pocc[OSLAMK_POCC_WORDS(base) + k] = s_occ[k];
         __syncthreads();
     }
 }
@@ -843,6 +870,13 @@
     return (int)hipGetLastError();
 }
 
+int oslamk_bucket_occupancy(oslamk_table t, oslamk_entries ent, void *stream)
+{
+    const size_t total = (size_t)t.n_slices * t.cap;
+    hipLaunchKernelGGL(k_bucket_occupancy, dim3((unsigned)total), dim3(SPREAD_THREADS), 0, (hipStream_t)stream, t, ent);
+    return (int)hipGetLastError();
+}
+
 int oslamk_reach_build(oslamk_table t, float d_dist, void *stream)
 {
     hipLaunchKernelGGL(k_reach_build, dim3(OSLAMK_REACH_BINS), dim3(256), 0, (hipStream_t)stream, t, d_dist);
diff --git a/objective-slam_amd/csrc/oslam_model.c b/objective-slam_amd/csrc/oslam_model.c
--- a/objective-slam_amd/csrc/oslam_model.c
+++ b/objective-slam_amd/csrc/oslam_model.c
@@ -15,6 +15,7 @@
     if (m->ent.pw) (void)hipFree(m->ent.pw);
     if (m->ent.puv) (void)hipFree(m->ent.puv);
     if (m->ent.pdir) (void)hipFree(m->ent.pdir);
+    if (m->ent.pocc) (void)hipFree(m->ent.pocc);
     if (m->ent.mi) (void)hipFree(m->ent.mi);
     if (m->table.ukeys && !m->shared_union) (void)hipFree(m->table.ukeys);
     if (m->table.reach && !m->shared_union) (void)hipFree(m->table.reach);
@@ -199,6 +200,17 @@
     return rc;
 }
 
+static int build_occupancy(oslam_model *m, size_t n_pairs)
+{
+    int rc = OSLAM_OK;
+    const size_t bytes = sizeof(uint32_t) * OSLAMK_POCC_WORDS(n_pairs + 256);
+    HIPCHK(hipMalloc((void **)&m->ent.pocc, bytes));
+    HIPCHK(hipMemsetAsync(m->ent.pocc, 0, bytes, (hipStream_t)oslam_stream()));
+    KCHK(oslamk_bucket_occupancy(m->table, m->ent, oslam_stream()));
+done:
+    return rc;
+}
+
 int oslam_model_create(const float *xyz, const float *nrm, size_t n, size_t stride_bytes,
                        float d_dist, const oslam_params *params, oslam_model **out)
 {
@@ -286,6 +298,8 @@
         HIPCHK(hipMalloc((void **)&m->ent.puv, sizeof(oslamk_uv) * n_pairs));
         HIPCHK(hipMalloc((void **)&m->ent.pdir, sizeof(uint16_t) * ((n_pairs + 256) << OSLAMK_PDIR_SHIFT)));
         KCHK(oslamk_bucket_psort(m->table, m->ent, oslam_stream()));
+        rc = build_occupancy(m, n_pairs);
+        if (rc != OSLAM_OK) goto done;
         HIPCHK(hipStreamSynchronize((hipStream_t)oslam_stream()));
         (void)hipFree(m->ent.uv);
         m->ent.uv = NULL;
@@ -524,6 +538,10 @@
     if (rc == OSLAM_OK && hd.has_uv) rc = db_read_dev(f, m->ent.pdir, sizeof(uint16_t) * ((size_t)hd.n_entries << OSLAMK_PDIR_SHIFT), &sum);
     if (rc != OSLAM_OK) goto done;
     if (sum != hd.checksum) { rc = fail(OSLAM_E_INVALID, "model file checksum mismatch"); goto done; }
+    if (hd.has_uv) {
+        rc = build_occupancy(m, n_pairs);
+        if (rc != OSLAM_OK) goto done;
+    }
     m->h_slots = h_slots;
     h_slots = NULL;
     rc = oslam_build_kmap(&m->table, m->d_dist, &m->table, 1, m->params.vote_order);
@@ -555,7 +573,8 @@
         *table_bytes = sizeof(oslamk_slot) * (uint64_t)m->table.cap * (uint64_t)m->table.n_slices +
                        sizeof(uint32_t) * (uint64_t)m->table.ucap + sizeof(uint32_t) * (OSLAMK_REACH_BINS / 32) +
                        sizeof(oslamk_uinfo) * (uint64_t)m->table.uinfo_stride * (uint64_t)m->table.n_slices +
-                       (uint64_t)m->n_entries * (4 + 2 + (m->ent.pw ? 12 + (2 << OSLAMK_PDIR_SHIFT) : 0)) + 24ull * (uint64_t)m->c.n;
+                       (uint64_t)m->n_entries * (4 + 2 + (m->ent.pw ? 12 + (2 << OSLAMK_PDIR_SHIFT) : 0)) +
+                       (m->ent.pocc ? sizeof(uint32_t) * (uint64_t)OSLAMK_POCC_WORDS(m->n_entries) : 0) + 24ull * (uint64_t)m->c.n;
     return OSLAM_OK;
 }
 
diff --git a/objective-slam_amd/csrc/oslam_taps.c b/objective-slam_amd/csrc/oslam_taps.c
--- a/objective-slam_amd/csrc/oslam_taps.c
+++ b/objective-slam_amd/csrc/oslam_taps.c
@@ -218,6 +218,14 @@
 {
     if (!acc_out) return fail(OSLAM_E_INVALID, "bad reference index");
     return tap_one_ref(m, s, ref_index, acc_out, NULL, NULL, NULL, 0, NULL, NULL);
+}
+
+int oslam_vote_edge_counts(const oslam_model *m, uint64_t *edge_votes, uint64_t *edge_candidates)
+{
+    if (!m) return fail(OSLAM_E_INVALID, "NULL handle");
+    if (edge_votes) *edge_votes = m->edge_votes;
+    if (edge_candidates) *edge_candidates = m->edge_candidates;
+    return OSLAM_OK;
 }
 
 int oslam_vote_hits(oslam_model *m, oslam_scene *s, size_t ref_index, uint32_t *numbers_out, uint32_t *theta_out,
diff --git a/objective-slam_amd/csrc/oslam_vote.c b/objective-slam_amd/csrc/oslam_vote.c
--- a/objective-slam_amd/csrc/oslam_vote.c
+++ b/objective-slam_amd/csrc/oslam_vote.c
@@ -251,6 +251,7 @@
     a->table.slots = m->table.slots;
     a->table.cap = m->table.cap;
     a->ent = m->ent;
+    if (m->params.no_edge_filter) a->ent.pocc = NULL;
     a->thresh = m->params.vote_count_threshold;
     a->counters = m->d_counters;
     a->out = m->d_out;
@@ -427,7 +428,12 @@
                             ? "a hit list overflowed: the counting pass and the hit pass disagreed on the pairs within reach"
                             : cnt[j].list_overflow & 2u ? "near-edge search: a hit's key number lies outside the model's bucket records"
                             : cnt[j].list_overflow & 4u ? "near-edge search: a bucket lies outside the model's entry arrays"
+                            : cnt[j].list_overflow & 16u ? "near-edge search: an occupancy word lies outside the model's entry arrays"
                                                         : "near-edge search: a directory place lies outside its bucket segment");
+    for (j = 0; j < v->nm; j++) {
+        v->ms[j]->edge_votes = cnt[j].edge_votes;
+        v->ms[j]->edge_candidates = cnt[j].edge_candidates;
+    }
     if (!t) return OSLAM_OK;
     HIPCHK(hipEventElapsedTime(&t->ms, ev[0], ev[1]));
     for (i = 0; i < pool->plan.nb && i < MAX_BATCH_EVENTS; i++) {
diff --git a/objective-slam_amd/csrc/oslam_vote_body.inc b/objective-slam_amd/csrc/oslam_vote_body.inc
--- a/objective-slam_amd/csrc/oslam_vote_body.inc
+++ b/objective-slam_amd/csrc/oslam_vote_body.inc
@@ -61,6 +61,7 @@
     const oslamk_pay *hits;
     const float *px, *py, *pz;
     const float *rows;
+    unsigned long long edge_counts;
     uint32_t inc_lo, inc_hi;
     uint32_t dropped;
 };
@@ -305,6 +306,7 @@
         s_ctx.inc_lo = PASS == 2 ? 0u : 1u;
         s_ctx.inc_hi = PASS == 0 ? 0x10000u : PASS == 2 ? 1u : 0u;
         s_ctx.dropped = 0;
+        s_ctx.edge_counts = 0;
     }
     const SlowCtx *sc = &s_ctx;
 
@@ -437,7 +439,7 @@
                 }
             }
         };
-        const uint32_t *skeys = a.hit_key + off;
+        const uint32_t *skeys = (const uint32_t *)uni_u64((unsigned long long)(a.hit_key + off));
         const uint32_t n_hits = a.hit_count[ref_local] < (uint32_t)(a.hit_off[ref_local + 1] - off) ? a.hit_count[ref_local]
                                                                                                    : (uint32_t)(a.hit_off[ref_local + 1] - off);
         const uint32_t n_cq = (n_hits + WAVE - 1u) / WAVE;
@@ -451,7 +453,9 @@
 #endif
             const uint32_t *pw = a.ent.pw;
             const uint16_t *pdir = a.ent.pdir;
+            const uint32_t *pocc = a.ent.pocc;
             const uint32_t hit = cq * WAVE + (uint32_t)lane;
+            uint32_t edge_v = 0, edge_c = 0;
             cq += VOTE_THREADS / WAVE;
             const bool in = hit < n_hits;
             const uint32_t kw = skeys[in ? hit : 0u];
@@ -466,11 +470,28 @@
             }
             const uint32_t A = pc_vote_base_t32(hits[in ? hit : 0u].theta_t22) * 30u - (PC_T24_EDGE - 1u), B = A + (PC_T24_EDGE - 1u);
             for (uint32_t seg = 0; __ballot(seg < ln); seg += OSLAMK_PSEG) {
-                const uint32_t n = seg < ln ? (ln - seg < OSLAMK_PSEG ? ln - seg : OSLAMK_PSEG) : 0u;
-                const uint32_t sbase = n ? ui.start + seg : 0u, K = OSLAMK_PDIR_CELLS(n);
+                const uint32_t n0 = seg < ln ? (ln - seg < OSLAMK_PSEG ? ln - seg : OSLAMK_PSEG) : 0u, s0 = n0 ? ui.start + seg : 0u;
+                bool live = n0 != 0u;
+                if (pocc) {
+                    const uint32_t Kf = pc_occ_cells(n0 << OSLAMK_POCC_SHIFT), fA = pc_occ_cell(A, Kf), fB = pc_occ_cell(B, Kf);
+                    const uint32_t w0 = (uint32_t)OSLAMK_POCC_WORDS(s0), iA = w0 + (fA >> 5), iB = w0 + (fB >> 5);
+                    const bool ld = n0 != 0u && (iA > iB ? iA : iB) < (uint32_t)OSLAMK_POCC_WORDS(a.ent.n_real);
+                    if (n0 != 0u && !ld) atomicOr(&a.counters->list_overflow, 16u);
+                    const uint32_t oA = ld ? pocc[iA] : 0u, oB = ld ? pocc[iB] : 0u;
+                    live = !pc_occ_clear(oA, fA, oB, fB);
+                }
+#ifdef VOTE_OCC_BESIDE
+                const uint32_t n = n0;
+#else
+                const uint32_t n = live ? n0 : 0u;
+#endif
+                const uint32_t sbase = n ? s0 : 0u, K = OSLAMK_PDIR_CELLS(n);
                 const uint32_t cA = __umulhi(A, K), cB = __umulhi(B, K);
                 const uint32_t d0 = n ? pdir[((size_t)sbase << OSLAMK_PDIR_SHIFT) + cA] : 0u, d1 = n ? pdir[((size_t)sbase << OSLAMK_PDIR_SHIFT) + cB + 1u] : 0u;
                 uint32_t cnt = K == 1u ? n : B < A ? n - d0 + d1 : d1 - d0;
+#ifdef VOTE_OCC_BESIDE
+                if (!live) cnt = 0;
+#endif
 #ifdef VOTE_DIAG_NOCAND
                 cnt = 0;
 #endif
@@ -485,6 +506,7 @@
                 }
                 const uint32_t excl = incl - cnt, total = readlane_u(incl, WAVE - 1);
                 const uint32_t hit0 = hit - (uint32_t)lane;
+                edge_c += total;
                 for (uint32_t base = 0; base < total; base += 4u * WAVE) {
                     uint32_t kk[4], own[4], w[4];
                     bool inl[4];
@@ -512,10 +534,12 @@
                         const uint32_t Ao = bperm(own[u], A);
                         const bool near = inl[u] && w[u] * 30u - Ao < PC_T24_EDGE;
                         const unsigned long long nm = __ballot(near);
+                        edge_v += (uint32_t)__popcll(nm);
                         if (nm) sq_n = slow_push((lds_ctx *)sc, (lds_u32 *)acc, (lds_u32 *)s_tbl, (lds_u64 *)sq, sq_n, nm, kk[u] | SLOW_VERIFY, (hit0 + own[u]) | (1u << SLOW_HIT_BITS), lane);
                     }
                 }
             }
+            if (lane == 0 && edge_c) atomicAdd(&s_ctx.edge_counts, ((unsigned long long)edge_c << 32) | edge_v);
 #ifdef VOTE_PROF
             prof_corr += clock64() - pc0;
 #endif
@@ -693,6 +717,10 @@
                         atomicAdd(&a.counters->entries, s_tot[1] & 0xffffffffffull);
                         atomicAdd(&a.counters->items, s_tot[1] >> 40);
                     }
+                    if (s_ctx.edge_counts) {
+                        atomicAdd(&a.counters->edge_votes, s_ctx.edge_counts & 0xffffffffull);
+                        atomicAdd(&a.counters->edge_candidates, s_ctx.edge_counts >> 32);
+                    }
                 }
                 uint32_t g = a.fixed_gmax;
                 if (g == 0) {
diff --git a/objective-slam_amd/csrc/ppf_core.h b/objective-slam_amd/csrc/ppf_core.h
--- a/objective-slam_amd/csrc/ppf_core.h
+++ b/objective-slam_amd/csrc/ppf_core.h
@@ -188,6 +188,20 @@
     return pc_alpha_bin_hybrid_ex(uy, uz, vy, vz, row, tbl, 0, 0);
 }
 
+#define PC_OCC_MIN_CELLS 32u
+#define PC_OCC_MAX_CELLS 4096u
+PM_HD uint32_t pc_occ_cells(uint32_t bits)
+{
+    return bits < 2u * PC_OCC_MIN_CELLS ? PC_OCC_MIN_CELLS : bits >= PC_OCC_MAX_CELLS ? PC_OCC_MAX_CELLS : 1u << (31 - __builtin_clz(bits));
+}
+PM_HD uint32_t pc_occ_cell(uint32_t P, uint32_t Kf) { return P >> (__builtin_clz(Kf) + 1); }
+PM_HD int pc_occ_clear(uint32_t wa, uint32_t ca, uint32_t wb, uint32_t cb) { return (((wa >> (ca & 31u)) | (wb >> (cb & 31u))) & 1u) == 0u; }
+PM_HD int pc_occ_rules_out(const uint32_t *seg_words, uint32_t Kf, uint32_t A, uint32_t B)
+{
+    const uint32_t ca = pc_occ_cell(A, Kf), cb = pc_occ_cell(B, Kf);
+    return pc_occ_clear(seg_words[ca >> 5], ca, seg_words[cb >> 5], cb);
+}
+
 #define PC_FAST_BOUND 3.1e-5
 PM_HD uint32_t pc_vote_base_fast_t32(uint32_t theta_v_t22) { return pc_vote_base_t32(theta_v_t22) - (PC_T24_MARGIN << 8); }
 PM_HD uint32_t pc_theta_fast(uint32_t theta_t22) { return theta_t22 == PC_T22_FORCE ? 0u : theta_t22; }
diff --git a/objective-slam_amd/ppf.py b/objective-slam_amd/ppf.py
--- a/objective-slam_amd/ppf.py
+++ b/objective-slam_amd/ppf.py
@@ -24,7 +24,7 @@
                 ("cpu_clustering", C.c_int), ("use_l1_norm", C.c_int), ("use_averaged_clusters", C.c_int),
                 ("dev", C.c_int), ("vote_mode", C.c_int), ("shard_rank", C.c_int), ("shard_world", C.c_int),
                 ("max_cells", C.c_uint), ("pose_gpu_min", C.c_uint), ("no_bucket_spread", C.c_int),
-                ("scratch_gib", C.c_uint), ("pose_two_sorts", C.c_int), ("vote_order", C.c_int), ("reserved", C.c_int * 1)]
+                ("scratch_gib", C.c_uint), ("pose_two_sorts", C.c_int), ("vote_order", C.c_int), ("no_edge_filter", C.c_int)]
 
 
 class Stats(C.Structure):
@@ -543,6 +543,7 @@
     "oslam_model_bucket": (_i, [_vp, C.c_uint32, _vp, _sz, C.POINTER(_sz)]),
     "oslam_model_bucket_words": (_i, [_vp, C.c_uint32, _i, _vp, _sz, C.POINTER(_sz)]),
     "oslam_vote_accumulator": (_i, [_vp, _vp, _sz, _vp]),
+    "oslam_vote_edge_counts": (_i, [_vp, C.POINTER(C.c_uint64), C.POINTER(C.c_uint64)]),
     "oslam_vote_hits": (_i, [_vp, _vp, _sz, _vp, _vp, _vp, _sz, C.POINTER(_sz), C.POINTER(C.c_uint32)]),
     "oslam_model_key_numbers": (_i, [_vp, _vp, _vp, _vp, _sz, C.POINTER(_sz)]),
     "oslam_vote_ref_order": (_i, [_vp, _sz, _vp]),
@@ -1139,6 +1140,12 @@
         w = np.ascontiguousarray(weights, np.float32)
         _check(lib().oslam_model_set_point_weights(self._h, _p(w), len(w)))
 
+    def _with_edge_counts(self, d):
+        v, c = C.c_uint64(0), C.c_uint64(0)
+        _check(lib().oslam_vote_edge_counts(self._h, C.byref(v), C.byref(c)))
+        d["num_edge_votes"], d["num_edge_candidates"] = int(v.value), int(c.value)
+        return d
+
     def prepare(self, scene):
         _check(lib().oslam_align_prepare(self._h, scene._h))
 
@@ -1149,7 +1156,7 @@
         if not (allow_no_votes and rc == OSLAM_E_NO_VOTES):
             _check(rc)
         self.best_T = T.reshape(4, 4)
-        self.stats = st.asdict()
+        self.stats = self._with_edge_counts(st.asdict())
         return self.best_T
 
     def refine(self, scene, T=None, params=None):
@@ -1180,7 +1187,7 @@
                                          cap, C.byref(n), C.byref(st))
         if rc != OSLAM_E_NO_VOTES:
             _check(rc)
-        self.stats = st.asdict()
+        self.stats = self._with_edge_counts(st.asdict())
         return [out[k].astuple() for k in range(n.value)]
 
     def align_local(self, scene, cap=None):
@@ -1189,11 +1196,11 @@
         st = Stats()
         if cap is None:
             _check(lib().oslam_align_local(self._h, scene._h, None, 0, C.byref(n), C.byref(lmax), C.byref(st)))
-            self.stats = st.asdict()
+            self.stats = self._with_edge_counts(st.asdict())
             return int(n.value), int(lmax.value)
         cells = np.zeros(cap, CELL_DTYPE)
         _check(lib().oslam_align_local(self._h, scene._h, _p(cells), cap, C.byref(n), C.byref(lmax), C.byref(st)))
-        self.stats = st.asdict()
+        self.stats = self._with_edge_counts(st.asdict())
         return cells[: n.value].copy(), int(lmax.value)
 
     def local_peaks(self, global_max):
@@ -1212,7 +1219,7 @@
         if not (allow_no_votes and rc == OSLAM_E_NO_VOTES):
             _check(rc)
         self.best_T = T.reshape(4, 4)
-        self.stats = st.asdict()
+        self.stats = self._with_edge_counts(st.asdict())
         return self.best_T
 
     def align_finish(self, scene, cells, global_max, allow_no_votes=False):
```

Result: no change. 26.12 billion scene PPFs/s (median of 3 runs) (-0.1%).
